# rslmtoasa/rslmtoasa

Hardware: AMD Instinct MI355X
Metric: block-recursion throughput (H|psi> + A_n + B_n recursion levels, recursion.f90 recur_b) (higher is better)
Workload: dtype f64

## Files before the change

include/rsrec.h:

```cpp
#ifndef RSREC_H
#define RSREC_H

#include <stddef.h>
#include <stdint.h>

#ifdef __cplusplus
extern "C" {
#endif

typedef struct rsrec_handle rsrec_t;

#define RSREC_OK 0
#define RSREC_ERR_ARG 1
#define RSREC_ERR_DEVICE 2
#define RSREC_ERR_DIVERGED 3
#define RSREC_ERR_EIG 4

int rsrec_version(void);

int rsrec_device_count(void);

int rsrec_create(rsrec_t **out, int device);
int rsrec_destroy(rsrec_t *h);

// ... 61 lines not shown

#define RSREC_LATTICE_NGROUP_MAX 16
int rsrec_chebyshev_lattice(rsrec_t *h, int nchains, int nseed, const int32_t *seed_atoms, const double *seed_coef, int lld, double a, double b,
                            int ngroup, const int32_t *group, double *m_g);

int rsrec_kubo_moments(rsrec_t *h, int nvec, int nseed, const int32_t *seed_atoms, const double *seed_coef, int cond_ll, double a, double b,
                       const double *v_a, const double *vo_a, const double *v_b, const double *vo_b, double *mu_nm);

int rsrec_kubo_moments_diag(rsrec_t *h, int nvec, int nseed, const int32_t *seed_atoms, const double *seed_coef, int cond_ll, double a, double b,
                            const double *v_a, const double *vo_a, const double *v_b, const double *vo_b, double *mu_diag);

#define RSREC_KUBO_NOUT_MAX 8
int rsrec_kubo_moments_diag_multi(rsrec_t *h, int nout, int nvec, int nseed, const int32_t *seed_atoms, const double *seed_coef,
                                  int cond_ll, double a, double b, const double *v_out, const double *vo_out, const double *v_b,
                                  const double *vo_b, double *mu_diag);

#define RSREC_KUBO_NIN_MAX 4
#define RSREC_KUBO_NSET_MAX 16
int rsrec_kubo_moments_diag_tensor(rsrec_t *h, int nin, int nout, int nvec, int nseed, const int32_t *seed_atoms, const double *seed_coef,
                                   int cond_ll, double a, double b, const double *v_out, const double *vo_out, const double *v_in,
                                   const double *vo_in, double *mu_diag);

#define RSREC_COND_LL_MAX 4096
int rsrec_kubo_integrand(rsrec_t *h, int nvec, int cond_ll, const double *mu_nm, int nen, const double *ene, double energy_min,
                         double energy_max, double *integrand);
int rsrec_kubo_integrand_diag(rsrec_t *h, int nvec, int cond_ll, const double *mu_diag, int nen, const double *ene, double energy_min,
                              double energy_max, double *integrand);

int rsrec_kubo_conductivity(rsrec_t *h, int nvec, int per_vector, int nen, int nv1, const double *ene, double energy_min, double energy_max,
                            double temperature, const double *integrand, double *sigma, double *series);

#define RSREC_OPT_NFERMI_MAX 16
int rsrec_kubo_optical(rsrec_t *h, int nset, int cond_ll, const double *mu_diag, int nen, const double *ene, double energy_min, double energy_max,
                       int nw, int nfermi, const double *fermi, double temperature, double *opt);

int rsrec_exchange(rsrec_t *h, int kind, int npairs, const int32_t *same, int lld, int nen, const double *ene, int nv1, double fermi,
                   int sym_term, double energy_min, double energy_max, const double *a_inf, const double *b_inf, const double *coef_a,
                   const double *coef_b, const double *dpar, int pair_offset, int npairs_total, double *xc, double *so, double *fo,
                   double *parts, double *jcum, double *integrand);

int rsrec_damping(rsrec_t *h, int kind, int npairs, const int32_t *same, int lld, int nen, const double *ene, int ief, int sym_term,
                  double energy_min, double energy_max, const double *a_inf, const double *b_inf, const double *coef_a, const double *coef_b,
                  const double *tmat, int pair_offset, int npairs_total, double *at_ef, double *total, double *rows);

int rsrec_exchange_aux(rsrec_t *h, int kind, int npairs, const int32_t *same, int lld, int nen, const double *ene, int nv1, double fermi,
                       int sym_term, double energy_min, double energy_max, const double *a_inf, const double *b_inf, const double *coef_a,
                       const double *coef_b, const double *apar, int pair_offset, int npairs_total, double *jaux, double *rows);

int rsrec_spin_lattice(rsrec_t *h, int kind, int npairs, const int32_t *same, int lld, int nen, const double *ene, int nv1, double fermi,
                       int sym_term, double energy_min, double energy_max, const double *a_inf, const double *b_inf, const double *coef_a,
                       const double *coef_b, const double *apar, const double *dmat, int trio_offset, int ntrios_total, double *jijk,
                       double *rows);

int rsrec_exchange_contour(rsrec_t *h, int kind, int npairs, const int32_t *same, int lld, int npts, const double *x, const double *w, double e0,
                           int sym_term, double energy_min, double energy_max, const double *a_inf, const double *b_inf, const double *coef_a,
                           const double *coef_b, const double *dmat, int pair_offset, int npairs_total, double *xc, double *rows);

int rsrec_contour_occupation(rsrec_t *h, int kind, int nsites, int lld, int npts, const double *x, const double *w, double e0, int sym_term,
                             double energy_min, double energy_max, const double *a_inf, const double *b_inf, const double *coef_a,
                             const double *coef_b, int site_offset, int nsites_total, double *occ, double *gdiag);

int rsrec_apply_operator(rsrec_t *h, int vel, const double *v_op, const double *vo_op, const double *psi_in, double *psi_out, double a, double b);

int rsrec_scalar_lanczos(rsrec_t *h, int nsites, const int32_t *seed_atoms, int lld, int llmax, double *a, double *b2);

void rsrec_site_partition(int rank, int nprocs, int nsites, int *start_atom, int *end_atom);

int rsrec_last_error(rsrec_t *h, char *buf, size_t n);

int rsrec_orbital_moments(rsrec_t *h, int nseeds, const int32_t *seed_atoms, int lld, double a, double b, const double *cr, double alat,
                          double *mu_orb, double *mu_seed);

int rsrec_pack_moments(rsrec_t *h, int site_offset, int nsites_total, double *mu_img);

#define RSREC_COMM_ID_BYTES 128
int rsrec_comm_unique_id(char *id);
int rsrec_comm_init(rsrec_t *h, int rank, int nranks, const char *id);
int rsrec_comm_init_file(rsrec_t *h, int rank, int nranks, const char *path, double timeout_s);
int rsrec_allreduce_sum(rsrec_t *h, double *buf, size_t n);
int rsrec_comm_size(rsrec_t *h, int *rank, int *nranks);
int rsrec_comm_destroy(rsrec_t *h);

int rsrec_set_option(rsrec_t *h, const char *key, long value);
int rsrec_get_timing(rsrec_t *h, double *out, int n);

#ifdef __cplusplus
}
#endif
#endif
```

rslmtoasa_amd/_lib.py:

```python
import ctypes as C
import os

_HERE = os.path.dirname(os.path.abspath(__file__))
LIB_PATH = os.environ.get("RSREC_LIB") or os.path.join(_HERE, "librsrec.so")

ERR_ARG, ERR_DEVICE, ERR_DIVERGED, ERR_EIG = 1, 2, 3, 4

_lib = None

_SIGNATURES = {
    "rsrec_version": (C.c_int, []),
    "rsrec_device_count": (C.c_int, []),
    "rsrec_create": (C.c_int, [C.POINTER(C.c_void_p), C.c_int]),
    "rsrec_destroy": (C.c_int, [C.c_void_p]),
    "rsrec_set_lattice": (C.c_int, [C.c_void_p, C.c_int, C.c_int, C.c_void_p, C.c_void_p, C.c_int, C.c_int]),
    "rsrec_set_positions": (C.c_int, [C.c_void_p, C.c_void_p]),
    "rsrec_set_hamiltonian": (C.c_int, [C.c_void_p, C.c_int, C.c_int, C.c_int] + [C.c_void_p] * 6),
    "rsrec_assemble_blocks": (C.c_int, [C.c_void_p, C.c_int, C.c_int, C.c_int, C.c_int, C.c_void_p, C.c_void_p, C.c_void_p, C.c_int, C.c_void_p, C.c_void_p]),
    "rsrec_block_lanczos": (C.c_int, [C.c_void_p, C.c_int, C.c_void_p, C.c_int, C.c_void_p, C.c_void_p]),
    "rsrec_block_lanczos_seeded": (C.c_int, [C.c_void_p, C.c_int, C.c_int, C.c_void_p, C.c_void_p, C.c_int, C.c_void_p, C.c_void_p]),
    "rsrec_block_lanczos_local_axis": (C.c_int, [C.c_void_p, C.c_int, C.c_void_p, C.c_void_p, C.c_int, C.c_void_p, C.c_void_p]),
    "rsrec_pack_diag": (C.c_int, [C.c_void_p, C.c_int, C.c_int, C.c_void_p, C.c_void_p]),
    "rsrec_orbital_moments": (C.c_int, [C.c_void_p, C.c_int, C.c_void_p, C.c_int, C.c_double, C.c_double, C.c_void_p, C.c_double, C.c_void_p, C.c_void_p]),
    "rsrec_pack_moments": (C.c_int, [C.c_void_p, C.c_int, C.c_int, C.c_void_p]),
    "rsrec_comm_unique_id": (C.c_int, [C.c_char_p]),
    "rsrec_comm_init": (C.c_int, [C.c_void_p, C.c_int, C.c_int, C.c_char_p]),
    "rsrec_comm_init_file": (C.c_int, [C.c_void_p, C.c_int, C.c_int, C.c_char_p, C.c_double]),
    "rsrec_allreduce_sum": (C.c_int, [C.c_void_p, C.c_void_p, C.c_size_t]),
    "rsrec_comm_size": (C.c_int, [C.c_void_p, C.POINTER(C.c_int), C.POINTER(C.c_int)]),
    "rsrec_comm_destroy": (C.c_int, [C.c_void_p]),
    "rsrec_terminator": (C.c_int, [C.c_void_p, C.c_int, C.c_int] + [C.c_void_p] * 6),
    "rsrec_scalar_density": (C.c_int, [C.c_void_p] + [C.c_int] * 4 + [C.c_void_p] * 2 + [C.c_int] + [C.c_void_p] * 4),
    "rsrec_block_ldos": (C.c_int, [C.c_void_p, C.c_int, C.c_void_p, C.c_double, C.c_double, C.c_int, C.c_int, C.c_int] + [C.c_void_p] * 5),
    "rsrec_kubo_moments": (C.c_int, [C.c_void_p, C.c_int, C.c_int, C.c_void_p, C.c_void_p, C.c_int, C.c_double, C.c_double] + [C.c_void_p] * 5),
    "rsrec_kubo_moments_diag": (C.c_int, [C.c_void_p, C.c_int, C.c_int, C.c_void_p, C.c_void_p, C.c_int, C.c_double, C.c_double] + [C.c_void_p] * 5),
    "rsrec_kubo_moments_diag_multi": (C.c_int, [C.c_void_p, C.c_int, C.c_int, C.c_int, C.c_void_p, C.c_void_p, C.c_int, C.c_double, C.c_double] + [C.c_void_p] * 5),
    "rsrec_kubo_moments_diag_tensor": (C.c_int, [C.c_void_p, C.c_int, C.c_int, C.c_int, C.c_int, C.c_void_p, C.c_void_p, C.c_int, C.c_double, C.c_double] + [C.c_void_p] * 5),
    "rsrec_exchange": (C.c_int, [C.c_void_p, C.c_int, C.c_int, C.c_void_p, C.c_int, C.c_int, C.c_void_p, C.c_int, C.c_double, C.c_int, C.c_double, C.c_double]
                       + [C.c_void_p] * 5 + [C.c_int, C.c_int] + [C.c_void_p] * 6),
    "rsrec_damping": (C.c_int, [C.c_void_p, C.c_int, C.c_int, C.c_void_p, C.c_int, C.c_int, C.c_void_p, C.c_int, C.c_int, C.c_double, C.c_double]
                      + [C.c_void_p] * 5 + [C.c_int, C.c_int] + [C.c_void_p] * 3),
    "rsrec_exchange_aux": (C.c_int, [C.c_void_p, C.c_int, C.c_int, C.c_void_p, C.c_int, C.c_int, C.c_void_p, C.c_int, C.c_double, C.c_int, C.c_double, C.c_double]
                           + [C.c_void_p] * 5 + [C.c_int, C.c_int] + [C.c_void_p] * 2),
    "rsrec_spin_lattice": (C.c_int, [C.c_void_p, C.c_int, C.c_int, C.c_void_p, C.c_int, C.c_int, C.c_void_p, C.c_int, C.c_double, C.c_int, C.c_double, C.c_double]
                           + [C.c_void_p] * 6 + [C.c_int, C.c_int] + [C.c_void_p] * 2),
    "rsrec_exchange_contour": (C.c_int, [C.c_void_p, C.c_int, C.c_int, C.c_void_p, C.c_int, C.c_int, C.c_void_p, C.c_void_p, C.c_double, C.c_int, C.c_double,
                                         C.c_double] + [C.c_void_p] * 5 + [C.c_int, C.c_int] + [C.c_void_p] * 2),
    "rsrec_contour_occupation": (C.c_int, [C.c_void_p, C.c_int, C.c_int, C.c_int, C.c_int, C.c_void_p, C.c_void_p, C.c_double, C.c_int, C.c_double,
                                           C.c_double] + [C.c_void_p] * 4 + [C.c_int, C.c_int] + [C.c_void_p] * 2),
    "rsrec_kubo_integrand": (C.c_int, [C.c_void_p, C.c_int, C.c_int, C.c_void_p, C.c_int, C.c_void_p, C.c_double, C.c_double, C.c_void_p]),
    "rsrec_kubo_integrand_diag": (C.c_int, [C.c_void_p, C.c_int, C.c_int, C.c_void_p, C.c_int, C.c_void_p, C.c_double, C.c_double, C.c_void_p]),
    "rsrec_kubo_conductivity": (C.c_int, [C.c_void_p, C.c_int, C.c_int, C.c_int, C.c_int, C.c_void_p, C.c_double, C.c_double, C.c_double] + [C.c_void_p] * 3),
    "rsrec_kubo_optical": (C.c_int, [C.c_void_p, C.c_int, C.c_int, C.c_void_p, C.c_int, C.c_void_p, C.c_double, C.c_double, C.c_int, C.c_int, C.c_void_p,
                                     C.c_double, C.c_void_p]),
    "rsrec_apply_operator": (C.c_int, [C.c_void_p, C.c_int, C.c_void_p, C.c_void_p, C.c_void_p, C.c_void_p, C.c_double, C.c_double]),
    "rsrec_zsqr": (C.c_int, [C.c_void_p, C.c_int, C.c_void_p]),
    "rsrec_chebyshev_green": (C.c_int, [C.c_void_p, C.c_int, C.c_int, C.c_int, C.c_void_p, C.c_double, C.c_double, C.c_void_p, C.c_void_p]),
    "rsrec_chebyshev_ldos": (C.c_int, [C.c_void_p, C.c_int, C.c_void_p, C.c_double, C.c_double, C.c_int, C.c_int] + [C.c_void_p] * 3),
    "rsrec_block_spectra": (C.c_int, [C.c_void_p, C.c_int, C.c_void_p, C.c_int, C.c_void_p, C.c_double, C.c_double, C.c_int, C.c_int, C.c_int, C.c_void_p]),
    "rsrec_chebyshev_spectra": (C.c_int, [C.c_void_p, C.c_int, C.c_void_p, C.c_int, C.c_void_p, C.c_double, C.c_double, C.c_int, C.c_int, C.c_void_p]),
    "rsrec_spectra_integrals": (C.c_int, [C.c_void_p, C.c_int, C.c_void_p, C.c_int, C.c_void_p, C.c_int, C.c_void_p, C.c_int, C.c_int, C.c_double, C.c_double,
                                          C.c_double, C.c_int, C.c_int, C.c_int, C.c_void_p, C.c_void_p]),
    "rsrec_block_green": (C.c_int, [C.c_void_p, C.c_int, C.c_int, C.c_int, C.c_void_p, C.c_double, C.c_double, C.c_int] + [C.c_void_p] * 5),
    "rsrec_chebyshev": (C.c_int, [C.c_void_p, C.c_int, C.c_void_p, C.c_int, C.c_double, C.c_double, C.c_void_p]),
    "rsrec_chebyshev_seeded": (C.c_int, [C.c_void_p, C.c_int, C.c_int, C.c_void_p, C.c_void_p, C.c_int, C.c_double, C.c_double, C.c_void_p]),
    "rsrec_chebyshev_pairs_direct": (C.c_int, [C.c_void_p, C.c_int, C.c_void_p, C.c_int, C.c_double, C.c_double, C.c_int, C.c_void_p, C.c_void_p]),
    "rsrec_chebyshev_bloch": (C.c_int, [C.c_void_p, C.c_int, C.c_void_p, C.c_int, C.c_double, C.c_double, C.c_void_p, C.c_void_p, C.c_int, C.c_void_p, C.c_int, C.c_void_p, C.c_void_p]),
    "rsrec_chebyshev_lattice": (C.c_int, [C.c_void_p, C.c_int, C.c_int, C.c_void_p, C.c_void_p, C.c_int, C.c_double, C.c_double, C.c_int, C.c_void_p, C.c_void_p]),
    "rsrec_scalar_lanczos":(C.c_int, [C.c_void_p, C.c_int, C.c_void_p, C.c_int, C.c_int, C.c_void_p, C.c_void_p]),
    "rsrec_site_partition": (None, [C.c_int, C.c_int, C.c_int, C.POINTER(C.c_int), C.POINTER(C.c_int)]),
    "rsrec_last_error": (C.c_int, [C.c_void_p, C.c_char_p, C.c_size_t]),
    "rsrec_set_option": (C.c_int, [C.c_void_p, C.c_char_p, C.c_long]),
    "rsrec_get_timing": (C.c_int, [C.c_void_p, C.POINTER(C.c_double), C.c_int]),
}


def exported_symbols():
    return sorted(_SIGNATURES)


def lib():
    global _lib
    if _lib is None:
        if not os.path.exists(LIB_PATH):
            raise RuntimeError("librsrec.so not built: run `make -C rslmtoasa_amd/csrc` (or __graft_entry__.build()); "
                               "there is no CPU fallback for the recursion engine")
        L = C.CDLL(LIB_PATH)
        for name, (res, args) in _SIGNATURES.items():
            fn = getattr(L, name)
            fn.restype = res
            fn.argtypes = args
        _lib = L
    return _lib


class RsrecError(RuntimeError):
    def __init__(self, code, msg):
        super().__init__("rsrec error %d: %s" % (code, msg))
        self.code = code
```

rslmtoasa_amd/csrc/kernels_uscheme.hpp:

```cpp
#pragma once
#include "kernels_mfma.hpp"
#include "kernels_spmm5.hpp"

namespace rsrec {

__host__ __device__ constexpr int pk_col(int q, int l4) { return q < 8 ? 8 * (q >> 1) + 2 * l4 + (q & 1) : 32 + l4; }

__device__ __forceinline__ void emit_rhs_frags_pk(const double2* M, double sign, double* out, int ci_layout) {
    for (int e = threadIdx.x; e < 27 * 64; e += blockDim.x) {
        const int l = e & 63, qf = e >> 6, q = qf / 3, f = qf % 3;
        const int ki = pk_col(q, l >> 4);
        const int ko = (f < 2) ? 16 * f + (l & 15) : 32 + (l & 3);
        const int pi = ci_layout ? (ki & 1) : ki / 18, ci = ci_layout ? (ki >> 1) : ki % 18;
        const int po = ci_layout ? (ko & 1) : ko / 18, co = ci_layout ? (ko >> 1) : ko % 18;
        const double2 g = M[ci + 18 * co];
        const double v = (pi == po) ? g.x : (pi == 0 ? g.y : -g.y);
        out[e] = sign * v;
    }
}

__device__ __forceinline__ void matmul18(const double2* A, const double2* B, double2* C) {
    for (int e = threadIdx.x; e < BLK; e += blockDim.x) {
        const int i = e % NB, j = e / NB;
        double2 acc = make_double2(0.0, 0.0);
        for (int k = 0; k < NB; ++k) {
            const double2 a = A[i + NB * k], b = B[k + NB * j];
            acc.x += a.x * b.x - a.y * b.y;
            acc.y += a.x * b.y + a.y * b.x;
        }
        C[e] = acc;
    }
}

struct U3Operands { double2 x[4]; double2 y; };

__device__ __forceinline__ void u3_load(U3Operands& o, const double* __restrict__ base, unsigned off, int l4) {
    const double2* p = reinterpret_cast<const double2*>(base + off + 2 * l4);
#pragma unroll
    for (int qq = 0; qq < 4; ++qq) o.x[qq] = ld_stream(p + 4 * qq);
    o.y = ld_stream(reinterpret_cast<const double2*>(base + off + 32 + 2 * (l4 >> 1)));
}

template <int Q>
__device__ __forceinline__ double u3_k(const U3Operands& o, bool odd) { return Q < 8 ? ((Q & 1) ? o.x[Q >> 1].y : o.x[Q >> 1].x) : (odd ? o.y.y : o.y.x); }

__device__ __forceinline__ void u3_mac(double4_t& ca, double4_t& cb, double& cr, const U3Operands& o, const double (&T)[27], bool odd) {
#define U3_STEP(Q)                                                                              \
    {                                                                                           \
        const double a = u3_k<Q>(o, odd);                                                          \
        ca = __builtin_amdgcn_mfma_f64_16x16x4f64(a, T[3 * (Q) + 0], ca, 0, 0, 0);              \
        cb = __builtin_amdgcn_mfma_f64_16x16x4f64(a, T[3 * (Q) + 1], cb, 0, 0, 0);              \
        cr = __builtin_amdgcn_mfma_f64_4x4x4f64(a, T[3 * (Q) + 2], cr, 0, 0, 0);                \
    }
    U3_STEP(0) U3_STEP(1) U3_STEP(2) U3_STEP(3) U3_STEP(4) U3_STEP(5) U3_STEP(6) U3_STEP(7) U3_STEP(8)
#undef U3_STEP
}

__global__ __launch_bounds__(MF_WAVES * 64, 1) void k_mfma_orth3(ChainView CV, int level, int zero_block, const double* __restrict__ tvec,
                                                                const double* __restrict__ ucur, double* uprev,
                                                                const double* __restrict__ tabs, double* partial ,
                                                                double* unext = nullptr ) {
    __shared__ double lds[MF_WAVES * 1296];
    const int chain = blockIdx.y;
    const int lane = threadIdx.x & 63;
    const int wave = __builtin_amdgcn_readfirstlane(threadIdx.x >> 6);
    const int ngroups = CV.count_of(chain, level) / GROUP;
    const int* order = CV.order_of(chain, level);
    const size_t vo = (size_t)chain * CV.vstride;
    const double* tv = tvec + vo;
    const double* uc = ucur + vo;
    double* up = uprev + vo;
    double* uo = (unext ? unext : uprev) + vo;
    const int l15 = lane & 15, l4 = lane >> 4, l3 = lane & 3, lg = (lane >> 2) & 3;
    double T1[27], T2[27], T3[27];
    {
        const double* f = tabs + (size_t)chain * 3 * 27 * 64 + lane;
#pragma unroll
        for (int e = 0; e < 27; ++e) { T1[e] = f[e * 64]; T2[e] = f[(27 + e) * 64]; T3[e] = f[(54 + e) * 64]; }
    }
    GramAcc Gm;
    Gm.zero();
    const int nbx = active_workgroups(ngroups);
    GroupWalk w((int)blockIdx.x < nbx ? ngroups : 0, wave, nbx);
    const int ntile = (w.g < w.end) ? ((w.end - w.g + w.step - 1) / w.step) * 9 : 0;
    struct TileAtoms { int s0, a_lo, a_hi; };
    auto tile_atoms = [&](int it) {
        it = min(it, ntile - 1);
        const int* __restrict__ grp = order + (size_t)(w.g + (it / 9) * w.step) * GROUP;
        TileAtoms t;
        t.s0 = (16 * (it % 9)) / 18;
        t.a_lo = grp[t.s0];
        t.a_hi = grp[min(t.s0 + 1, GROUP - 1)];
        return t;
    };
    auto tile_row = [&](const TileAtoms& t, int rho) {
        const bool hi = rho >= 18 * (t.s0 + 1);
        const int a = hi ? t.a_hi : t.a_lo;
        RowRef R;
        R.valid = a >= 0;
        R.off = (unsigned)BLD * (unsigned)(R.valid ? a : zero_block) + 36u * (unsigned)(rho - 18 * (t.s0 + (hi ? 1 : 0)));
        return R;
    };
    auto load_tile = [&](int it, U3Operands& a, U3Operands& c, U3Operands& p) {
        const TileAtoms t = tile_atoms(it);
        const RowRef ra = tile_row(t, 16 * (min(it, ntile - 1) % 9) + l15);
        u3_load(a, tv, ra.off, l4);
        u3_load(c, uc, ra.off, l4);
        u3_load(p, up, ra.off, l4);
    };
    struct Pending { double4_t ca, cb; double cr; TileAtoms ta; int mt; };
    Pending P;
    bool pending = false;
    auto retire = [&](const double (&fr)[4]) {
#pragma unroll
        for (int j = 0; j < 4; ++j) {
            const RowRef rs = tile_row(P.ta, 16 * P.mt + l4 + 4 * j);
            if (rs.valid) { st_stream(uo + rs.off + l15, (double)P.ca[j]); st_stream(uo + rs.off + 16 + l15, (double)P.cb[j]); }
        }
        const RowRef rr = tile_row(P.ta, 16 * P.mt + 4 * lg + l4);
        if (rr.valid) st_stream(uo + rr.off + 32 + l3, P.cr);
#pragma unroll
        for (int j = 0; j < 4; ++j) {
            const double f0 = P.ca[j], f1 = P.cb[j];
            Gm.t00 = __builtin_amdgcn_mfma_f64_16x16x4f64(f0, f0, Gm.t00, 0, 0, 0);
            Gm.t01 = __builtin_amdgcn_mfma_f64_16x16x4f64(f0, f1, Gm.t01, 0, 0, 0);
            Gm.t11 = __builtin_amdgcn_mfma_f64_16x16x4f64(f1, f1, Gm.t11, 0, 0, 0);
            Gm.tr0 = __builtin_amdgcn_mfma_f64_4x4x4f64(fr[j], f0, Gm.tr0, 0, 0, 0);
            Gm.tr1 = __builtin_amdgcn_mfma_f64_4x4x4f64(fr[j], f1, Gm.tr1, 0, 0, 0);
            Gm.trr = __builtin_amdgcn_mfma_f64_4x4x4f64(fr[j], fr[j], Gm.trr, 0, 0, 0);
        }
    };
    auto compute_tile = [&](int it, const U3Operands& ot, const U3Operands& oc, const U3Operands& op) {
        double fr[4] = {0.0, 0.0, 0.0, 0.0};
        if (pending) {
#pragma unroll
            for (int j = 0; j < 4; ++j) fr[j] = __shfl(P.cr, l3 + 4 * j + 16 * l4, 64);
        }
        Pending N;
        N.ta = tile_atoms(it);
        N.mt = it % 9;
        N.ca = (double4_t){0, 0, 0, 0}; N.cb = (double4_t){0, 0, 0, 0}; N.cr = 0.0;
        u3_mac(N.ca, N.cb, N.cr, ot, T1, l4 & 1);
        if (pending) retire(fr);
        u3_mac(N.ca, N.cb, N.cr, op, T2, l4 & 1);
        u3_mac(N.ca, N.cb, N.cr, oc, T3, l4 & 1);
        P = N;
        pending = true;
    };
    U3Operands at, ac, ap, bt, bc, bp, ct, cc, cp;
    if (ntile > 0) { load_tile(0, at, ac, ap); load_tile(1, bt, bc, bp); }
#pragma unroll 1
    for (int it = 0; it < ntile; it += 3) {
        load_tile(it + 2, ct, cc, cp);
        __builtin_amdgcn_sched_barrier(0);
        compute_tile(it, at, ac, ap);
        __builtin_amdgcn_sched_barrier(0);
        if (it + 1 < ntile) {
            load_tile(it + 3, at, ac, ap);
            __builtin_amdgcn_sched_barrier(0);
            compute_tile(it + 1, bt, bc, bp);
            __builtin_amdgcn_sched_barrier(0);
        }
        if (it + 2 < ntile) {
            load_tile(it + 4, bt, bc, bp);
            __builtin_amdgcn_sched_barrier(0);
            compute_tile(it + 2, ct, cc, cp);
            __builtin_amdgcn_sched_barrier(0);
        }
    }
    if (pending) {
        double fr[4];
#pragma unroll
        for (int j = 0; j < 4; ++j) fr[j] = __shfl(P.cr, l3 + 4 * j + 16 * l4, 64);
        retire(fr);
    }
    gram_block_out(Gm, lds, partial + ((size_t)chain * gridDim.x + blockIdx.x) * 1296, true);
}

template <int F>
__device__ __forceinline__ void u3_mac_lds(double4_t& ca, double4_t& cb, double& cr, const U3Operands& o, const double* __restrict__ T , bool odd) {
#define U3L_STEP(Q)                                                                             \
    {                                                                                           \
        const double a = u3_k<Q>(o, odd);                                                          \
        ca = __builtin_amdgcn_mfma_f64_16x16x4f64(a, T[(3 * (Q) + 0) * 64], ca, 0, 0, 0);       \
        cb = __builtin_amdgcn_mfma_f64_16x16x4f64(a, T[(3 * (Q) + 1) * 64], cb, 0, 0, 0);       \
        cr = __builtin_amdgcn_mfma_f64_4x4x4f64(a, T[(3 * (Q) + 2) * 64], cr, 0, 0, 0);         \
    }
    U3L_STEP(0) U3L_STEP(1) U3L_STEP(2) U3L_STEP(3) U3L_STEP(4) U3L_STEP(5) U3L_STEP(6) U3L_STEP(7) U3L_STEP(8)
#undef U3L_STEP
}

__global__ __launch_bounds__(MF_WAVES * 64, 2) void k_mfma_orth3w(ChainView CV, int level, int zero_block, const double* __restrict__ tvec,
                                                                 const double* __restrict__ ucur, double* uprev,
                                                                 const double* __restrict__ tabs, double* partial ) {
    __shared__ double lds[MF_WAVES * 1296];
    const int chain = blockIdx.y;
    const int lane = threadIdx.x & 63;
    const int wave = __builtin_amdgcn_readfirstlane(threadIdx.x >> 6);
    const int ngroups = CV.count_of(chain, level) / GROUP;
    const int* order = CV.order_of(chain, level);
    const size_t vo = (size_t)chain * CV.vstride;
    const double* tv = tvec + vo;
    const double* uc = ucur + vo;
// ... 271 lines not shown
```

rslmtoasa_amd/csrc/rsrec.hip:

```cpp
#include <hip/hip_runtime.h>
#include <hsa/hsa.h>
#include <hsa/hsa_ext_amd.h>
#include <dlfcn.h>
#include <algorithm>
#include <array>
#include <atomic>
#include <chrono>
#include <cmath>
#include <cstdarg>
#include <cstdio>
#include <cstdlib>
#include <cstring>
#include <memory>
#include <string>
#include <thread>
#include <tuple>
#include <vector>

#include "../../include/rsrec.h"
#include "kernels_valu.hpp"
#include "kernels_mfma.hpp"
#include "kernels_spmm4.hpp"
#include "kernels_spmm5.hpp"
#include "kernels_uscheme.hpp"
#include "kernels_green.hpp"
#include "kernels_ldos.hpp"
#include "kernels_spectra.hpp"
#include "kernels_moments.hpp"
#include "kernels_kubo.hpp"
#include "kernels_cond.hpp"
#include "kernels_optical.hpp"
#include "kernels_exchange.hpp"
#include "kernels_auxgreen.hpp"
#include "kernels_contour.hpp"
#include "kernels_assemble.hpp"
#include "kernels_fan.hpp"
#include "kernels_bloch.hpp"
#include "kernels_lattice.hpp"

using namespace rsrec;

namespace {

struct DevBuf {
    void* p = nullptr;
    size_t bytes = 0;
    DevBuf() = default;
    DevBuf(DevBuf&& o) noexcept : p(o.p), bytes(o.bytes) { o.p = nullptr; o.bytes = 0; }
    DevBuf& operator=(DevBuf&& o) noexcept { std::swap(p, o.p); std::swap(bytes, o.bytes); return *this; }
    ~DevBuf() { release(); }
    hipError_t reserve(size_t n) {
        if (n <= bytes) return hipSuccess;
        release();
        hipError_t e = hipMalloc(&p, n);
        if (e == hipSuccess) bytes = n;
        return e;
    }
    void release() { if (p) (void)hipFree(p); p = nullptr; bytes = 0; }
    template <class T> T* as() const { return reinterpret_cast<T*>(p); }
};

}

struct rsrec_handle {
    int device = 0;
    hipStream_t stream = nullptr;
    hipStream_t copy_stream = nullptr;
    hipEvent_t ev_green[2] = {nullptr, nullptr};
    hipStream_t side_stream = nullptr;
    hipEvent_t ev_orth = nullptr, ev_bred = nullptr;
    hipStream_t oct_stream = nullptr;
    hipEvent_t ev_oct_in = nullptr, ev_oct_out = nullptr;
    size_t p2_slot = 0;
    std::string err;
    bool have_lattice = false, have_ham = false;
    std::vector<int32_t> lat_nn, lat_iz;
    int lat_nncols = 0;
    std::vector<double> lat_cr;
    int kk = 0, nslots = 0, nmax = 0, ntype = 0;
    std::vector<int> nbr;
    std::vector<int> iz0;
    std::vector<int> radj_ptr, radj;
    DevBuf d_nbr, d_iz, d_nbr5;
    int hslots = 0, hoh = 0, nsp = 2;
    DevBuf d_hst, d_hloc, d_host, d_holoc, d_enim, d_lsham;
    Spmm4Operator s4_op;
    int s4_built_split = 0;
    Spmm5Operator s5_op;
    DevBuf d_s5queue;
    int s5_built = 0;
    size_t s5_lds_limit = (size_t)-1;
    int n_cu = 0;
    bool s4_attr = false;
    size_t term_lds = 0, cheb_ldos_lds = (size_t)64 * 1024, cheb_spec_lds = (size_t)64 * 1024;
    std::vector<double> host_ee, host_lsham, host_eeo, host_enim, host_hall, host_hallo;
    std::vector<double> host_st, host_loc;
    DevBuf d_asm[2][2], d_asm_in;
    std::vector<double> asm_host[2][2];
    int asm_nslots[2] = {0, 0}, asm_ncls[2] = {0, 0}, asm_hoh[2] = {0, 0};
    int n_octet_launch = 0;
    int n_asm_reused = 0;
    long n_asm_calls = 0, n_ldos_calls = 0, n_recursion_calls = 0;
    Spmm5Operator s5_la; int s5_la_ok = 0;
    DevBuf d_la_extra, d_rot;
    Spmm5Operator kubo_op[RSREC_KUBO_NOUT_MAX], kubo_op_b[RSREC_KUBO_NIN_MAX], kubo_hbulk;
    Spmm5Operator orb_plain;
    DevBuf d_green_in, d_green_out;
    DevBuf d_kubo[5];
    DevBuf d_cond[4];
    DevBuf d_ctens[2];
    DevBuf d_opt[5];
    DevBuf d_bsqrt, d_term, d_gim, d_ldos;
    DevBuf d_ops, d_spec;
    struct SpecImage { int nop = 0, nen = 0, n = 0, site_offset = 0, nsites_total = 0; } spec_res;
    DevBuf d_mint;
    void* pin = nullptr;
    size_t pin_bytes = 0;
    DevBuf d_frags, d_vec[6], d_partial, d_partial2, d_coefA, d_coefB, d_bmats, d_status, d_seed, d_seedcoef, d_mu, d_scal, d_zsqr;
    DevBuf d_fan, d_fan_tab, d_mpair;
    DevBuf d_bloch_geo, d_bloch_tab;
    DevBuf d_lat_tab, d_lat_w, d_lat_part;
    long opt_batch = 0, opt_kernels = 0, opt_nblk = 0, opt_spmm5 = 2, opt_chain_fold = 1, opt_s5_cap = 0, opt_side = 1, opt_s5_lds = 1, opt_s5_queue = 1, opt_cheb_fused = 1;
    long opt_s5_waves = 8;
    long opt_sat_pct = 100;
    long opt_orth_oop = 1;
    long opt_s5_split = 0;
    long opt_s5_run_min = 0;
    long opt_s5_spin_xcd = 0;
    long opt_s5_octet = 8;
    long opt_s5_host_emit = 0;
    long opt_kubo_lchunk = 0;
    long opt_kubo_vbatch = 0;
    long opt_lattice_vbatch = 0;
    long opt_kubo_setgroup = 0;
    int n_kubo_left_chunks = 0;
    int kubo_diag_nvec = 0, kubo_diag_ll = 0;
    long opt_orth3 = 1;
    long opt_graph = 1;
    long opt_s5_gram_min = 256;
    int ham_hermitian = 0;
    std::vector<int> opp_slot;
    int opp_epoch = -1;
    DevBuf d_gram;
    double n_gram_folded = 0, n_gram_all = 0, n_gram_levels = 0;
    hipGraphExec_t graph_exec = nullptr;
    std::vector<uintptr_t> graph_key;
    bool capturing = false;
    double t_total_ms = 0, t_hop_ms = 0, t_rest_ms = 0, t_host_ms = 0;
    double t_rot_ms = 0;
    double n_hop_launch = 0, n_atom_steps = 0, n_block_mult = 0, n_hop_mfma_flop = 0;
    double n_req_flop = 0;
    int hop_fuses_a = 1;
    std::vector<hipEvent_t> ev_pool;
    size_t ev_used = 0;
    struct RegionEntry {
        std::vector<int> seeds;
        int nlev, napply, flags, epoch, ostride;
        double atom_steps, block_mults;
        DevBuf order, cum;
        std::vector<int> level_max;
        std::vector<int> hop_min, hop_max;
        std::vector<double> level_groups;
        std::vector<double> mult_hist;
        struct ClassRun { int tau, lo, hi; };
        std::vector<ClassRun> sat_runs;
        std::vector<int> level_sat;
        int sat_base = 0;
    };
    std::vector<std::unique_ptr<RegionEntry>> region_cache;
    int lattice_epoch = 0;
    const int* cur_order = nullptr;
    const int* cur_cum = nullptr;
    const std::vector<int>* cur_level_max = nullptr;
    const std::vector<double>* cur_level_groups = nullptr;
    const std::vector<double>* cur_mult_hist = nullptr;
    const RegionEntry* cur_entry = nullptr;
    int cur_nrows = 0;
    std::vector<unsigned> spatial_key;
    int res_kind = 0, res_n = 0, res_lld = 0;
    bool res_seeded = false;
    void* comm = nullptr;
    int comm_rank = 0, comm_nranks = 1;
    DevBuf d_comm;
    ~rsrec_handle();
};

namespace {

struct OptionEntry { const char* name; long rsrec_handle::*member; };
const OptionEntry OPTIONS[] = {
    {"batch", &rsrec_handle::opt_batch},
    {"kernels", &rsrec_handle::opt_kernels},
    {"nblk", &rsrec_handle::opt_nblk},
    {"spmm5", &rsrec_handle::opt_spmm5},
    {"chain_fold", &rsrec_handle::opt_chain_fold},
    {"s5_cap", &rsrec_handle::opt_s5_cap},
    {"s5_lds", &rsrec_handle::opt_s5_lds},
    {"s5_queue", &rsrec_handle::opt_s5_queue},
    {"cheb_fused", &rsrec_handle::opt_cheb_fused},
    {"side_stream", &rsrec_handle::opt_side},
    {"graph", &rsrec_handle::opt_graph},
    {"orth3", &rsrec_handle::opt_orth3},
    {"s5_waves", &rsrec_handle::opt_s5_waves},
    {"s5_split", &rsrec_handle::opt_s5_split},
    {"orth_oop", &rsrec_handle::opt_orth_oop},
    {"sat_pct", &rsrec_handle::opt_sat_pct},
    {"kubo_lchunk", &rsrec_handle::opt_kubo_lchunk},
    {"kubo_vbatch", &rsrec_handle::opt_kubo_vbatch},
    {"kubo_setgroup", &rsrec_handle::opt_kubo_setgroup},
    {"lattice_vbatch", &rsrec_handle::opt_lattice_vbatch},
    {"s5_host_emit", &rsrec_handle::opt_s5_host_emit},
    {"s5_octet", &rsrec_handle::opt_s5_octet},
    {"s5_spin_xcd", &rsrec_handle::opt_s5_spin_xcd},
    {"s5_run_min", &rsrec_handle::opt_s5_run_min},
    {"s5_gram_min", &rsrec_handle::opt_s5_gram_min},
};

int fail(rsrec_t* h, int code, const char* fmt, ...) {
    char buf[512];
    va_list ap;
    va_start(ap, fmt);
    vsnprintf(buf, sizeof buf, fmt, ap);
    va_end(ap);
    if (h) h->err = buf;
    return code;
}

#define HIPCK(h, call)                                                                                         \
    do {                                                                                                       \
        hipError_t e_ = (call);                                                                                \
        if (e_ != hipSuccess) return fail(h, RSREC_ERR_DEVICE, "%s failed: %s (%s:%d)", #call, hipGetErrorString(e_), __FILE__, __LINE__); \
    } while (0)

hipEvent_t next_event(rsrec_t* h) {
    static const bool off = getenv("RSREC_NO_EVENTS") != nullptr;
    if (off || h->capturing) return nullptr;
    if (h->ev_used == h->ev_pool.size()) {
        hipEvent_t e;
        if (hipEventCreate(&e) != hipSuccess) return nullptr;
        h->ev_pool.push_back(e);
    }
    hipEvent_t e = h->ev_pool[h->ev_used++];
    (void)hipEventRecord(e, h->stream);
    return e;
}

constexpr size_t PIN_BYTES = (size_t)8 << 20;
int pin_ready(rsrec_t* h) {
    if (h->pin) return RSREC_OK;
    if (hipHostMalloc(&h->pin, PIN_BYTES, hipHostMallocDefault) != hipSuccess) { h->pin = nullptr; return fail(h, RSREC_ERR_DEVICE, "hipHostMalloc of the staging buffer failed"); }
    h->pin_bytes = PIN_BYTES;
    return RSREC_OK;
}
constexpr size_t PIN_MAX_XFER = (size_t)8 << 20;
int xfer_d2h(rsrec_t* h, void* dst, const void* src_dev, size_t bytes) {
    if (bytes > PIN_MAX_XFER) {
        HIPCK(h, hipMemcpyAsync(dst, src_dev, bytes, hipMemcpyDeviceToHost, h->stream));
        HIPCK(h, hipStreamSynchronize(h->stream));
        return RSREC_OK;
    }
    int rc = pin_ready(h);
    if (rc) return rc;
    for (size_t off = 0; off < bytes; off += h->pin_bytes) {
        const size_t n = std::min(h->pin_bytes, bytes - off);
        HIPCK(h, hipMemcpyAsync(h->pin, static_cast<const char*>(src_dev) + off, n, hipMemcpyDeviceToHost, h->stream));
        HIPCK(h, hipStreamSynchronize(h->stream));
        memcpy(static_cast<char*>(dst) + off, h->pin, n);
    }
    return RSREC_OK;
}
int xfer_h2d(rsrec_t* h, void* dst_dev, const void* src, size_t bytes) {
    if (bytes > PIN_MAX_XFER) {
        HIPCK(h, hipMemcpyAsync(dst_dev, src, bytes, hipMemcpyHostToDevice, h->stream));
        HIPCK(h, hipStreamSynchronize(h->stream));
        return RSREC_OK;
    }
    int rc = pin_ready(h);
    if (rc) return rc;
    for (size_t off = 0; off < bytes; off += h->pin_bytes) {
        const size_t n = std::min(h->pin_bytes, bytes - off);
        memcpy(h->pin, static_cast<const char*>(src) + off, n);
        HIPCK(h, hipMemcpyAsync(static_cast<char*>(dst_dev) + off, h->pin, n, hipMemcpyHostToDevice, h->stream));
        HIPCK(h, hipStreamSynchronize(h->stream));
    }
    return RSREC_OK;
}
#define XFER(call) do { int rc__ = (call); if (rc__) return rc__; } while (0)

// ... 60 lines not shown
void spatial_key_from_graph(rsrec_t* h) {
    const int kk = h->kk;
    std::vector<int> d0, d1, d2;
    bfs_dist(h, 0, d0);
    int l1 = 0;
    for (int i = 0; i < kk; ++i) if (d0[i] >= d0[l1]) l1 = i;
    bfs_dist(h, l1, d1);
    int l2 = 0, best = -1;
    for (int i = 0; i < kk; ++i) { const int m = std::min(d0[i], d1[i]); if (m >= best) { best = m; l2 = i; } }
    bfs_dist(h, l2, d2);
    h->spatial_key.resize(kk);
    for (int i = 0; i < kk; ++i) h->spatial_key[i] = morton3((unsigned)std::max(d0[i], 0), (unsigned)std::max(d1[i], 0), (unsigned)std::max(d2[i], 0));
}

}

extern "C" int rsrec_version(void) { return 101; }

extern "C" int rsrec_device_count(void) {
    int n = 0;
    if (hipGetDeviceCount(&n) != hipSuccess) return 0;
    return n;
}

static rsrec_handle* g_report_handle = nullptr;
static void report_at_exit() {
    const rsrec_handle* h = g_report_handle;
    if (!h) return;
    std::printf("rsrec report: library_calls=%ld device_assemblies=%ld operator_arrays_from_device=%d device_ldos_calls=%ld\n", h->n_recursion_calls, h->n_asm_calls,
                h->n_asm_reused, h->n_ldos_calls);
    std::fflush(stdout);
}

extern "C" int rsrec_create(rsrec_t** out, int device) {
    if (!out) return RSREC_ERR_ARG;
    *out = nullptr;
    int ndev = 0;
    if (hipGetDeviceCount(&ndev) != hipSuccess || ndev <= 0) return RSREC_ERR_DEVICE;
    if (device < 0 || device >= ndev) return RSREC_ERR_ARG;
    if (hipSetDevice(device) != hipSuccess) return RSREC_ERR_DEVICE;
    rsrec_t* h = new rsrec_handle();
    h->device = device;
    if (hipStreamCreateWithFlags(&h->stream, hipStreamNonBlocking) != hipSuccess) { delete h; return RSREC_ERR_DEVICE; }
    if (hipDeviceGetAttribute(&h->n_cu, hipDeviceAttributeMultiprocessorCount, device) != hipSuccess || h->n_cu <= 0) h->n_cu = 256;
    *out = h;
    if (getenv("RSREC_REPORT") && !g_report_handle) {
        static bool registered = false;
        if (!registered) { registered = std::atexit(report_at_exit) == 0; }
        g_report_handle = h;
    }
    return RSREC_OK;
}

rsrec_handle::~rsrec_handle() {
    (void)hipSetDevice(device);
    if (stream) (void)hipStreamSynchronize(stream);
    if (graph_exec) (void)hipGraphExecDestroy(graph_exec);
    (void)rsrec_comm_destroy(this);
    for (hipEvent_t e : ev_pool) (void)hipEventDestroy(e);
    for (hipStream_t s : {stream, copy_stream, side_stream, oct_stream}) if (s) (void)hipStreamDestroy(s);
    for (hipEvent_t e : {ev_green[0], ev_green[1], ev_orth, ev_bred, ev_oct_in, ev_oct_out}) if (e) (void)hipEventDestroy(e);
    if (pin) (void)hipHostFree(pin);
}

extern "C" int rsrec_destroy(rsrec_t* h) {
    if (!h) return RSREC_ERR_ARG;
    if (g_report_handle == h) { report_at_exit(); g_report_handle = nullptr; }
    delete h;
    return RSREC_OK;
}

extern "C" int rsrec_last_error(rsrec_t* h, char* buf, size_t n) {
    if (!h || !buf || n == 0) return RSREC_ERR_ARG;
    snprintf(buf, n, "%s", h->err.c_str());
    return RSREC_OK;
}

extern "C" int rsrec_set_option(rsrec_t* h, const char* key, long value) {
    if (!h || !key) return RSREC_ERR_ARG;
    for (const OptionEntry& o : OPTIONS)
        if (!strcmp(key, o.name)) { h->*o.member = value; return RSREC_OK; }
    return fail(h, RSREC_ERR_ARG, "unknown option '%s'", key);
}

extern "C" int rsrec_get_timing(rsrec_t* h, double* out, int n) {
    if (!h || !out) return RSREC_ERR_ARG;
    const double v[14] = {h->t_total_ms, h->t_hop_ms, h->n_hop_launch, h->n_atom_steps, h->n_block_mult, h->t_rest_ms, h->t_host_ms, (double)h->hop_fuses_a, h->n_hop_mfma_flop,
                          h->n_req_flop, (double)h->n_asm_reused, (double)h->n_octet_launch, h->t_rot_ms, h->n_gram_folded};
    for (int i = 0; i < n && i < 14; ++i) out[i] = v[i];
    return RSREC_OK;
}

extern "C" void rsrec_site_partition(int rank, int nprocs, int nsites, int* start_atom, int* end_atom) {
    int per = nsites / nprocs;
    const int rem = nsites % nprocs;
    int start;
    if (rank < rem) { per += 1; start = rank * per + 1; }
    else start = rank * per + rem + 1;
    *start_atom = start;
    *end_atom = start + per - 1;
}

static void release_graph(rsrec_t* h) {
    if (h->graph_exec) { (void)hipDeviceSynchronize(); (void)hipGraphExecDestroy(h->graph_exec); h->graph_exec = nullptr; }
    h->graph_key.clear();
}

static void release_regions(rsrec_t* h) {
    release_graph(h);
    if (!h->region_cache.empty()) (void)hipDeviceSynchronize();
    h->region_cache.clear();
    h->cur_order = nullptr; h->cur_cum = nullptr; h->cur_entry = nullptr; h->cur_level_max = nullptr; h->cur_level_groups = nullptr; h->cur_mult_hist = nullptr;
}

extern "C" int rsrec_set_lattice(rsrec_t* h, int kk, int nncols, const int32_t* nn, const int32_t* iz, int nmax, int ntype) {
    if (!h || !nn || !iz || kk <= 0 || nncols < 1 || nmax < 0 || nmax > kk || ntype < 1) return fail(h, RSREC_ERR_ARG, "rsrec_set_lattice: bad argument");
    HIPCK(h, hipSetDevice(h->device));
    if (h->have_lattice && kk == h->kk && nncols == h->lat_nncols && nmax == h->nmax && ntype == h->ntype &&
        h->lat_nn.size() == (size_t)kk * nncols && std::memcmp(h->lat_nn.data(), nn, h->lat_nn.size() * sizeof(int32_t)) == 0 &&
        std::memcmp(h->lat_iz.data(), iz, (size_t)kk * sizeof(int32_t)) == 0)
        return RSREC_OK;
    int nslots = 1;
    for (int i = 0; i < kk; ++i) {
        const int nr = nn[i];
        if (nr < 0 || nr > nncols) return fail(h, RSREC_ERR_ARG, "rsrec_set_lattice: nn(%d,1)=%d outside 0..%d", i + 1, nr, nncols);
        nslots = std::max(nslots, nr);
        if (iz[i] < 1 || iz[i] > ntype) return fail(h, RSREC_ERR_ARG, "rsrec_set_lattice: iz(%d)=%d outside 1..%d", i + 1, iz[i], ntype);
    }
    std::vector<int> nbr_new((size_t)kk * nslots, -1), iz_new(kk), deg(kk + 1, 0);
    for (int i = 0; i < kk; ++i) {
        iz_new[i] = iz[i] - 1;
        nbr_new[(size_t)i * nslots] = i;
        const int nr = nn[i];
        for (int j = 1; j < nr; ++j) {
            const int n = nn[(size_t)i + (size_t)kk * j];
            if (n == 0) continue;
            if (n < 0 || n > kk) return fail(h, RSREC_ERR_ARG, "rsrec_set_lattice: nn(%d,%d)=%d outside 0..%d", i + 1, j + 1, n, kk);
            nbr_new[(size_t)i * nslots + j] = n - 1;
            deg[n - 1]++;
        }
    }
    h->have_lattice = false;
    h->have_ham = false;
    h->kubo_diag_nvec = h->kubo_diag_ll = 0;
    h->lat_nn.clear(); h->lat_iz.clear();
    release_regions(h);
    h->kk = kk; h->nslots = nslots; h->nmax = nmax; h->ntype = ntype;
    h->nbr.swap(nbr_new);
    h->iz0.swap(iz_new);
    h->radj_ptr.assign(kk + 1, 0);
    for (int n = 0; n < kk; ++n) h->radj_ptr[n + 1] = h->radj_ptr[n] + deg[n];
    h->radj.resize(h->radj_ptr[kk]);
    std::vector<int> fill(h->radj_ptr.begin(), h->radj_ptr.end() - 1);
    for (int i = 0; i < kk; ++i)
        for (int j = 1; j < nslots; ++j) {
            const int n = h->nbr[(size_t)i * nslots + j];
            if (n >= 0) h->radj[fill[n]++] = i;
        }
    HIPCK(h, h->d_nbr.reserve(h->nbr.size() * sizeof(int)));
    HIPCK(h, h->d_iz.reserve((size_t)kk * sizeof(int)));
    HIPCK(h, hipMemcpy(h->d_nbr.p, h->nbr.data(), h->nbr.size() * sizeof(int), hipMemcpyHostToDevice));
    HIPCK(h, hipMemcpy(h->d_iz.p, h->iz0.data(), (size_t)kk * sizeof(int), hipMemcpyHostToDevice));
    {
        std::vector<int> n5((size_t)(kk + 1) * (nslots + 2), kk);
        for (int i = 0; i < kk; ++i) {
            for (int j = 0; j < nslots; ++j) { const int n = h->nbr[(size_t)i * nslots + j]; if (n >= 0) n5[(size_t)i * (nslots + 2) + j] = n; }
// ... 121 lines not shown
        if (dev && !hoh) k_fold_onsite<<<ntype, 324, 0, h->stream>>>(h->d_hst.as<double2>(), nslots, h->d_lsham.as<double2>(), nullptr);
    }
    std::vector<double> loc;
    if (nmax > 0) {
        loc.assign(hall, hall + B * nslots * nmax);
        if (!hoh)
            for (int i = 0; i < nmax; ++i)
                for (size_t e = 0; e < B; ++e) loc[B * nslots * i + e] += lsham[B * h->iz0[i] + e];
        const double* dev = resident(1, 0, hall, nmax);
        HIPCK(h, place(h->d_hloc, dev, loc.data(), loc.size()));
        if (dev && !hoh) k_fold_onsite<<<nmax, 324, 0, h->stream>>>(h->d_hloc.as<double2>(), nslots, h->d_lsham.as<double2>(), h->d_iz.as<int>());
    }
    if (hoh) {
        HIPCK(h, place(h->d_host, resident(0, 1, eeo, ntype), eeo, B * nslots * ntype));
        HIPCK(h, h->d_enim.reserve(B * ntype * 8));
        HIPCK(h, hipMemcpy(h->d_enim.p, enim, B * ntype * 8, hipMemcpyHostToDevice));
        if (nmax > 0) HIPCK(h, place(h->d_holoc, resident(1, 1, hallo, nmax), hallo, B * nslots * nmax));
    }
    HIPCK(h, hipGetLastError());
    {
        h->s4_built_split = 0; h->s5_built = 0;
        if (h->nslots + 1 <= S4_MAXSLOTS) {
            h->host_st.swap(st);
            h->host_loc.swap(loc);
            const double* dev[6] = {h->d_hst.as<double>(), h->d_hloc.as<double>(), h->d_host.as<double>(), h->d_holoc.as<double>(), h->d_enim.as<double>(), h->d_lsham.as<double>()};
            const char* msg = h->s5_op.build(h->nslots, nslots, ntype, nmax, h->hoh, h->host_st.data(), nmax > 0 ? h->host_loc.data() : nullptr, hoh ? eeo : nullptr,
                                             (hoh && nmax > 0) ? hallo : nullptr, hoh ? enim : nullptr, lsham, h->iz0.data(), h->opt_s5_host_emit ? nullptr : dev, h->stream);
            if (msg) return fail(h, RSREC_ERR_DEVICE, "rsrec_set_hamiltonian: %s", msg);
            h->s5_built = 1;
        }
    }
    h->have_ham = true;
    return RSREC_OK;
}

extern "C" int rsrec_assemble_blocks(rsrec_t* h, int part, int ncls, int nslots, int hoh, const double* hmag, const int32_t* nbr_type, const double* obarm, int ntype,
                                     double* blocks, double* blocks_o) {
    if (!h) return RSREC_ERR_ARG;
    if (part < 0 || part > 1 || ncls < 1 || nslots < 1 || !hmag || !blocks) return fail(h, RSREC_ERR_ARG, "rsrec_assemble_blocks: part=%d ncls=%d nslots=%d or a missing array", part, ncls, nslots);
    if (hoh && (!nbr_type || !obarm || !blocks_o || ntype < 1)) return fail(h, RSREC_ERR_ARG, "rsrec_assemble_blocks: hoh needs nbr_type, obarm (ntype=%d) and blocks_o", ntype);
    if (hoh)
        for (size_t q = 0; q < (size_t)ncls * nslots; ++q)
            if (nbr_type[q] < 0 || nbr_type[q] > ntype) return fail(h, RSREC_ERR_ARG, "rsrec_assemble_blocks: nbr_type[%zu]=%d outside 0..%d", q, nbr_type[q], ntype);
    HIPCK(h, hipSetDevice(h->device));
    h->n_asm_calls++;
    h->asm_nslots[part] = h->asm_ncls[part] = 0;
    const size_t nblk = (size_t)ncls * nslots, hm_bytes = nblk * 4 * 81 * 16, ty_bytes = nblk * 4, ob_bytes = hoh ? (size_t)ntype * 324 * 16 : 0;
    const size_t ty_off = (hm_bytes + 255) / 256 * 256, ob_off = ty_off + (ty_bytes + 255) / 256 * 256;
    HIPCK(h, h->d_asm_in.reserve(ob_off + ob_bytes + 256));
    char* in = h->d_asm_in.as<char>();
    XFER(xfer_h2d(h, in, hmag, hm_bytes));
    if (hoh) { XFER(xfer_h2d(h, in + ty_off, nbr_type, ty_bytes)); XFER(xfer_h2d(h, in + ob_off, obarm, ob_bytes)); }
    HIPCK(h, h->d_asm[part][0].reserve(nblk * 324 * 16));
    if (hoh) HIPCK(h, h->d_asm[part][1].reserve(nblk * 324 * 16));
    k_assemble_blocks<<<dim3(nslots, ncls), 384, 0, h->stream>>>(reinterpret_cast<const double2*>(in), reinterpret_cast<const int*>(in + ty_off),
                                                                 reinterpret_cast<const double2*>(in + ob_off), nslots, hoh ? 1 : 0, h->d_asm[part][0].as<double2>(),
                                                                 hoh ? h->d_asm[part][1].as<double2>() : nullptr);
    HIPCK(h, hipGetLastError());
    XFER(xfer_d2h(h, blocks, h->d_asm[part][0].p, nblk * 324 * 16));
    if (hoh) XFER(xfer_d2h(h, blocks_o, h->d_asm[part][1].p, nblk * 324 * 16));
    h->asm_host[part][0].assign(blocks, blocks + nblk * 648);
    if (hoh) h->asm_host[part][1].assign(blocks_o, blocks_o + nblk * 648); else h->asm_host[part][1].clear();
    h->asm_nslots[part] = nslots; h->asm_ncls[part] = ncls; h->asm_hoh[part] = hoh ? 1 : 0;
    return RSREC_OK;
}

namespace {

DevProblem make_problem(const rsrec_t* h) {
    DevProblem P;
    P.kk = h->kk; P.nslots = h->nslots; P.hstride = h->hslots; P.nmax = h->nmax; P.hoh = h->hoh;
    P.nbr = h->d_nbr.as<int>(); P.iz = h->d_iz.as<int>();
    P.h_st = h->d_hst.as<double2>(); P.h_loc = h->d_hloc.as<double2>();
    P.ho_st = h->d_host.as<double2>(); P.ho_loc = h->d_holoc.as<double2>();
    P.enim = h->d_enim.as<double2>(); P.lsham = h->d_lsham.as<double2>();
    return P;
}

void release_kubo_buffers(rsrec_t* h, bool moments, bool integrand) {
    if (moments) { for (auto& kb : h->d_kubo) kb.release(); h->kubo_diag_nvec = h->kubo_diag_ll = 0; }
    if (integrand) { for (auto& cb : h->d_cond) cb.release(); for (auto& cb : h->d_ctens) cb.release(); for (auto& cb : h->d_opt) cb.release(); }
}

struct BatchPlan {
    int batch = 1, nblk = 1;
};

int plan_batch(rsrec_t* h, int nchains, int nvec, size_t vec_elems_per_chain, BatchPlan& bp, size_t extra_bytes_per_chain = 0) {
    release_kubo_buffers(h, true, true);
    size_t free_b = 0, total_b = 0;
    HIPCK(h, hipMemGetInfo(&free_b, &total_b));
    size_t reusable = 0;
    for (int v = 0; v < 5; ++v) reusable += h->d_vec[v].bytes;
    if (extra_bytes_per_chain) reusable += h->d_gram.bytes;
    const double per_chain = (double)nvec * vec_elems_per_chain * sizeof(double2) + (double)h->kk * 4 + 4096 + (double)extra_bytes_per_chain;
    long cap = (long)((0.85 * (double)(free_b + reusable)) / per_chain);
    if (cap < 1) return fail(h, RSREC_ERR_DEVICE, "not enough device memory for one chain (%.1f MB needed, %.1f MB free)", per_chain / 1e6, free_b / 1e6);
    long b = h->opt_batch > 0 ? h->opt_batch : 64;
    b = std::min<long>(b, cap);
    b = std::min<long>(b, nchains);
    bp.batch = (int)std::max<long>(b, 1);
    long nblk = h->opt_nblk > 0 ? h->opt_nblk : std::max<long>(2048 / bp.batch, 16);
    nblk = std::min<long>(nblk, 256);
    nblk = std::min<long>(nblk, (h->kk + TILE_ATOMS - 1) / TILE_ATOMS);
    bp.nblk = (int)std::max<long>(nblk, 1);
    return RSREC_OK;
}

int upload_regions(rsrec_t* h, const int* seeds0, int nb, int nseed, int nlev, int napply, bool two_pass, bool grouped, int& ostride,
                   double& atom_steps, double& block_mults) {
    const int kk = h->kk;
    const int cap = grouped ? kk + 7 * h->nmax + 7 * h->ntype + 8 : kk;
    const int cap_pre = ((grouped ? kk + 7 * h->nmax + 7 * h->ntype * nlev + 8 : kk) + GROUP - 1) / GROUP * GROUP;
    const int flags = (two_pass ? 1 : 0) | (grouped ? 2 : 0) | ((int)std::min<long>(100, std::max<long>(1, h->opt_sat_pct)) << 2) | (nseed << 9);
    for (const auto& e : h->region_cache)
        if (e->epoch == h->lattice_epoch && e->nlev == nlev && e->napply == napply && e->flags == flags && (int)e->seeds.size() == nb * nseed &&
            std::equal(e->seeds.begin(), e->seeds.end(), seeds0)) {
            h->cur_order = e->order.as<int>(); h->cur_cum = e->cum.as<int>(); h->cur_nrows = nb; h->cur_level_max = &e->level_max; h->cur_level_groups = &e->level_groups;
            h->cur_mult_hist = &e->mult_hist;
            h->cur_entry = e.get();
            ostride = e->ostride;
            atom_steps += e->atom_steps; block_mults += e->block_mults;
            return RSREC_OK;
        }
    const int ntau_h = h->nmax + h->ntype, nfs_h = h->nslots + 1;
    const int sat_pct = (int)std::min<long>(100, std::max<long>(1, h->opt_sat_pct));
    const int sat_from = (int)(((long)sat_pct * kk + 99) / 100);
    std::vector<Region> regs(nb);
    auto run_threads = [&](auto&& fn) {
        const int nthr = std::max(1, std::min({nb, 8, (int)std::thread::hardware_concurrency()}));
        if (nthr == 1) { for (int c = 0; c < nb; ++c) fn(c); return; }
        std::atomic<int> next_chain{0};
        std::vector<std::thread> pool;
        for (int t = 0; t < nthr; ++t)
            pool.emplace_back([&]() { for (int c = next_chain++; c < nb; c = next_chain++) fn(c); });
        for (auto& th : pool) th.join();
    };
    run_threads([&](int c) { grow_region(h, seeds0 + (size_t)c * nseed, nseed, nlev, regs[c]); });
    size_t lvneed = 8;
    for (int c = 0; c < nb; ++c) {
        size_t need = 0;
        for (int L = 0; L < nlev; ++L) {
            const int n = regs[c].cum[L];
            if (n >= sat_from || (L > 0 && n == regs[c].cum[L - 1])) continue;
            need += (size_t)n + (grouped ? (size_t)7 * std::min(ntau_h, n) + 8 : 0);
        }
        lvneed = std::max(lvneed, need);
    }
    lvneed = (lvneed + 7) / 8 * 8;
    if (lvneed + (size_t)cap > (size_t)INT32_MAX) return fail(h, RSREC_ERR_ARG, "region lists of %zu entries per chain exceed the index range", lvneed + (size_t)cap);
    if ((size_t)cap_pre + lvneed + (size_t)cap > (size_t)INT32_MAX) return fail(h, RSREC_ERR_ARG, "region lists of %zu entries per chain exceed the index range", (size_t)cap_pre + lvneed + (size_t)cap);
    const int sat_off = cap_pre + (int)lvneed;
    ostride = sat_off + cap;
    std::vector<int> order((size_t)nb * ostride, -1), cum((size_t)4 * nb * nlev, 0);
    std::vector<double> as(nb, 0.0), bm(nb, 0.0);
    const size_t hist_n = (size_t)2 * ntau_h * nfs_h;
    std::vector<double> hist((size_t)nb * hist_n, 0.0);
    auto tau = [&](int i) { return i < h->nmax ? i : h->nmax + h->iz0[i]; };
    const std::vector<unsigned>& key = h->spatial_key;
    auto before = [&](int x, int y) {
        const int tx = grouped ? tau(x) : 0, ty = grouped ? tau(y) : 0;
        if (tx != ty) return tx < ty;
        if (key[x] != key[y]) return key[x] < key[y];
        return x < y;
    };
    std::vector<int> all(kk), sat_list;
    for (int i = 0; i < kk; ++i) all[i] = i;
    std::sort(all.begin(), all.end(), before);
    sat_list.reserve(cap);
    for (int q = 0; q < kk; ++q) {
        if (grouped && q > 0 && tau(all[q]) != tau(all[q - 1])) while (sat_list.size() % GROUP) sat_list.push_back(-1);
        sat_list.push_back(all[q]);
    }
    if (grouped) while (sat_list.size() % GROUP) sat_list.push_back(-1);
    const int sat_count = (int)sat_list.size();
    std::vector<double> lgroups((size_t)nb * nlev * ntau_h, 0.0);
    auto build_chain = [&](int c) {
        const Region& R = regs[c];
        int* orow = order.data() + (size_t)c * ostride;
        int* crow = cum.data() + (size_t)c * nlev;
        int* brow = cum.data() + (size_t)(nb + c) * nlev;
        int* crow2 = cum.data() + (size_t)(2 * nb + c) * nlev;
        int* brow2 = cum.data() + (size_t)(3 * nb + c) * nlev;
        std::copy(sat_list.begin(), sat_list.end(), orow + sat_off);
        int w = cap_pre, wp = 0;
        std::vector<int> lev, region, merged;
        for (int L = 0; L < nlev; ++L) {
            const int lo = L ? R.cum[L - 1] : 0, hi = R.cum[L];
            if (hi >= sat_from) { crow[L] = crow2[L] = sat_count; brow[L] = brow2[L] = sat_off; continue; }
            lev.assign(R.order.begin() + lo, R.order.begin() + hi);
            std::sort(lev.begin(), lev.end(), before);
            for (size_t q = 0; q < lev.size(); ++q) {
                if (grouped && q > 0 && tau(lev[q]) != tau(lev[q - 1])) while (wp % GROUP) orow[wp++] = -1;
                orow[wp++] = lev[q];
            }
            if (grouped) while (wp % GROUP) orow[wp++] = -1;
            crow2[L] = wp; brow2[L] = 0;
            if (L > 0 && hi == lo) { crow[L] = crow[L - 1]; brow[L] = brow[L - 1]; continue; }
            merged.resize(region.size() + lev.size());
            std::merge(region.begin(), region.end(), lev.begin(), lev.end(), merged.begin(), before);
            region.swap(merged);
            brow[L] = w;
            double* G = lgroups.data() + ((size_t)c * nlev + L) * ntau_h;
            for (size_t q = 0; q < region.size(); ++q) {
                if (grouped && q > 0 && tau(region[q]) != tau(region[q - 1])) while (w % GROUP) orow[w++] = -1;
                if (w % GROUP == 0) G[grouped ? tau(region[q]) : 0] += 1.0;
                orow[w++] = region[q];
            }
            if (grouped) while (w % GROUP) orow[w++] = -1;
            crow[L] = w - brow[L];
        }
        double a_s = 0.0, b_m = 0.0;
        for (int t = 1; t <= napply; ++t) {
            const int lv_after = two_pass ? 2 * t : t;
            a_s += R.cum[std::min(lv_after, nlev - 1)];
        }
        std::vector<int> lev_of(kk, -1);
        {
            int lv = 0;
            for (int q = 0; q < R.cum[nlev - 1]; ++q) {
                while (q >= R.cum[lv]) ++lv;
                lev_of[R.order[q]] = lv;
            }
        }
        std::vector<double> uses1(nlev + 1, 0.0), uses2(nlev + 1, 0.0);
        for (int d = 0; d < nlev; ++d)
            for (int t = 1; t <= napply; ++t) {
                if (!two_pass) { if (d <= t - 1) uses1[d] += 1.0; }
                else { if (d <= 2 * (t - 1)) uses1[d] += 1.0; if (d <= 2 * t - 1) uses2[d] += 1.0; }
            }
        double* H = hist.data() + (size_t)c * hist_n;
        const int ns = h->nslots;
        for (int i = 0; i < kk; ++i) {
            const int ti = tau(i);
            for (int s = 0; s < ns; ++s) {
                const int n = h->nbr[(size_t)i * ns + s];
                if (n < 0 || lev_of[n] < 0) continue;
                H[(size_t)ti * nfs_h + s] += uses1[lev_of[n]];
                if (two_pass) H[((size_t)ntau_h + ti) * nfs_h + s] += uses2[lev_of[n]];
            }
            if (two_pass && lev_of[i] >= 0) H[((size_t)ntau_h + ti) * nfs_h + ns] += uses1[lev_of[i]];
        }
        for (size_t q = 0; q < hist_n; ++q) b_m += H[q];
        if (two_pass) for (int t2 = 0; t2 < ntau_h; ++t2) b_m += H[((size_t)ntau_h + t2) * nfs_h + ns];
        as[c] = a_s; bm[c] = b_m;
    };
    run_threads(build_chain);
    double as_sum = 0.0, bm_sum = 0.0;
    for (int c = 0; c < nb; ++c) { as_sum += as[c]; bm_sum += bm[c]; }
    atom_steps += as_sum; block_mults += bm_sum;
    if (h->region_cache.size() >= 256) {
        HIPCK(h, hipStreamSynchronize(h->stream));
        h->region_cache.clear();
        h->cur_entry = nullptr;
    }
    h->region_cache.push_back(std::make_unique<rsrec_handle::RegionEntry>());
    rsrec_handle::RegionEntry* e = h->region_cache.back().get();
    e->seeds.assign(seeds0, seeds0 + (size_t)nb * nseed);
    e->nlev = nlev; e->napply = napply; e->flags = flags; e->epoch = h->lattice_epoch; e->ostride = ostride;
    e->atom_steps = as_sum; e->block_mults = bm_sum;
    e->mult_hist.assign(hist_n, 0.0);
    for (int c = 0; c < nb; ++c)
        for (size_t q = 0; q < hist_n; ++q) e->mult_hist[q] += hist[(size_t)c * hist_n + q];
    HIPCK(h, e->order.reserve(order.size() * 4));
    HIPCK(h, e->cum.reserve(cum.size() * 4));
    XFER(xfer_h2d(h, e->order.p, order.data(), order.size() * 4));
    XFER(xfer_h2d(h, e->cum.p, cum.data(), cum.size() * 4));
    HIPCK(h, hipStreamSynchronize(h->stream));
    e->level_max.assign(nlev, 0);
    e->hop_min.assign(nlev, INT32_MAX); e->hop_max.assign(nlev, 0);
    e->level_groups.assign((size_t)nlev * ntau_h, 0.0);
    {
        std::vector<double> sat_hist(ntau_h, 0.0);
        for (int g = 0; g < sat_count / GROUP; ++g) sat_hist[tau(sat_list[(size_t)g * GROUP])] += 1.0;
        e->sat_base = sat_off;
        e->level_sat.assign(nlev, 0);
        if (grouped)
            for (int g = 0; g < sat_count / GROUP; ++g) {
                const int t = tau(sat_list[(size_t)g * GROUP]);
                if (e->sat_runs.empty() || e->sat_runs.back().tau != t) e->sat_runs.push_back({t, g, g + 1});
                else e->sat_runs.back().hi = g + 1;
            }
        for (int c = 0; c < nb; ++c) {
            const double* prev = nullptr;
            for (int l = 0; l < nlev; ++l) {
                const int cnt = cum[(size_t)c * nlev + l];
                e->level_max[l] = std::max(e->level_max[l], cnt);
                e->hop_min[l] = std::min(e->hop_min[l], cnt); e->hop_max[l] = std::max(e->hop_max[l], cnt);
                const bool sat = cum[(size_t)(nb + c) * nlev + l] == sat_off;
                e->level_max[l] = std::max(e->level_max[l], cum[(size_t)(2 * nb + c) * nlev + l]);
                if (sat) e->level_sat[l] += 1;
                const double* G = lgroups.data() + ((size_t)c * nlev + l) * ntau_h;
                if (!sat && l > 0 && cum[(size_t)(nb + c) * nlev + l] == cum[(size_t)(nb + c) * nlev + l - 1] && prev) G = prev;
                for (int t2 = 0; t2 < ntau_h; ++t2) e->level_groups[(size_t)l * ntau_h + t2] += sat ? sat_hist[t2] : G[t2];
                prev = sat ? nullptr : G;
            }
        }
    }
    h->cur_order = e->order.as<int>(); h->cur_cum = e->cum.as<int>(); h->cur_nrows = nb; h->cur_level_max = &e->level_max; h->cur_level_groups = &e->level_groups;
    h->cur_mult_hist = &e->mult_hist;
    h->cur_entry = e;
    return RSREC_OK;
}

double required_hop_flops(const rsrec_t* h, const Spmm5Operator& op) {
    if (!h->cur_mult_hist) return 0.0;
    const int ntau = h->nmax + h->ntype, nfs = h->nslots + 1;
    const std::vector<double>& H = *h->cur_mult_hist;
    if (H.size() != (size_t)2 * ntau * nfs) return 0.0;
    double f = 0.0;
    for (int pass = 0; pass < 2; ++pass)
        for (int t = 0; t < ntau; ++t)
            for (int s = 0; s < nfs; ++s) {
                const double n = H[((size_t)pass * ntau + t) * nfs + s];
                if (n == 0.0) continue;
                const double w = (op.mixing.empty() || op.ntau != ntau || op.nslots != h->nslots) ? 46656.0 : op.required_flops(pass, t, s);
                f += n * (w > 0.0 ? w : 46656.0);
            }
    return f;
}

void reset_timing(rsrec_t* h) {
    h->t_total_ms = h->t_hop_ms = h->t_rest_ms = h->t_host_ms = h->t_rot_ms = 0;
    h->n_hop_launch = h->n_atom_steps = h->n_block_mult = h->n_hop_mfma_flop = h->n_req_flop = 0;
    h->n_octet_launch = 0;
    h->n_gram_folded = h->n_gram_all = h->n_gram_levels = 0;
    h->ev_used = 0;
    h->n_recursion_calls++;
}

// ... 239 lines not shown
int ensure_s4(rsrec_t* h) {
    if (h->s4_built_split) return RSREC_OK;
    const char* msg = h->s4_op.build(h->nslots, h->hslots, h->ntype, h->nmax, 0, h->host_st.data(), h->nmax > 0 ? h->host_loc.data() : nullptr, nullptr, nullptr, 1);
    if (msg) return fail(h, RSREC_ERR_DEVICE, "k_spmm4 operator tables: %s", msg);
    h->s4_built_split = 1;
    return RSREC_OK;
}

int s4_prepare(rsrec_t* h) {
    if (!h->s4_attr) {
        HIPCK(h, hipFuncSetAttribute(reinterpret_cast<const void*>(k_spmm4<4>), hipFuncAttributeMaxDynamicSharedMemorySize, (int)S4_LDS_BYTES));
        h->s4_attr = true;
    }
    return RSREC_OK;
}
int launch_spmm(rsrec_t* h, const SpmmDims& SD, const ChainView& CV, const DevProblem& P, int set, const double* in, double* out, dim3 grid_mf) {
    { const int rc = s4_prepare(h); if (rc) return rc; }
    dim3 g4(std::min<unsigned>(grid_mf.x * 4, 1024), grid_mf.y);
    k_spmm4<4><<<g4, MF_WAVES * 64, S4_LDS_BYTES, h->stream>>>(SD, CV.order, CV.cum, P.nbr, P.iz, h->s4_op.frag_set(set), h->s4_op.meta_set(set), in, out);
    return RSREC_OK;
}

__global__ __launch_bounds__(256) void k_rotate_coef(double2* __restrict__ A, double2* __restrict__ B, const double2* __restrict__ rot, int lld) {
#pragma clang fp contract(off)
    __shared__ double2 sM[BLK], sR[BLK], sT[BLK];
    const int chain = blockIdx.y, m = blockIdx.x;
    const bool is_a = m < lld - 1;
    double2* M = (is_a ? A : B) + ((size_t)chain * lld + (is_a ? m : m - (lld - 1) + 1)) * BLK;
    const double2* R = rot + (size_t)chain * BLK;
    for (int e = threadIdx.x; e < BLK; e += blockDim.x) { sM[e] = M[e]; sR[e] = R[e]; }
    __syncthreads();
    for (int e = threadIdx.x; e < BLK; e += blockDim.x) {
        const int i = e % NB, j = e / NB;
        double sr = 0.0, si = 0.0;
#pragma unroll
        for (int k = 0; k < NB; ++k) {
            const double ar = sM[i + NB * k].x, ai = sM[i + NB * k].y, br = sR[k + NB * j].x, bi = sR[k + NB * j].y;
            sr += ar * br - ai * bi; si += ar * bi + ai * br;
        }
        sT[e] = make_double2(sr, si);
    }
    __syncthreads();
    for (int e = threadIdx.x; e < BLK; e += blockDim.x) {
        const int i = e % NB, j = e / NB;
        double sr = 0.0, si = 0.0;
#pragma unroll
        for (int k = 0; k < NB; ++k) {
            const double ar = sR[k + NB * i].x, ai = -sR[k + NB * i].y, br = sT[k + NB * j].x, bi = sT[k + NB * j].y;
            sr += ar * br - ai * bi; si += ar * bi + ai * br;
        }
        M[e] = make_double2(sr, si);
    }
}

struct RecursionCall {
    bool mfma = false, side = false;
    int nchains = 0, nseed = 1, napply = 0, nlev = 0;
    const double* rot = nullptr;
    const Spmm5Operator* op = nullptr;
    int ci = 0;
    size_t velems = 0;
    int nvec = 0, skip_vec = -1, B = 1, nblk = 1;
    DevProblem P;
    hipEvent_t ev_begin = nullptr;
    std::vector<std::pair<hipEvent_t, hipEvent_t>> hop_ev, rot_ev;
};

RecursionCall recursion_call(const rsrec_t* h, bool mfma, int nchains, int nseed, int napply, const double* rot = nullptr) {
    RecursionCall RC;
    RC.mfma = mfma; RC.nchains = nchains; RC.nseed = nseed; RC.napply = napply; RC.rot = rot;
    RC.nlev = (h->hoh ? 2 * napply : napply) + 1; RC.op = rot ? &h->s5_la : &h->s5_op; RC.velems = (size_t)(h->kk + 1) * BLD;
    const bool large = (long)std::min(nchains, 64) * (h->kk / GROUP + 1) >= 4096;
    RC.ci = (mfma && (h->hoh || rot || h->opt_spmm5 == 2 || (h->opt_spmm5 == 1 && large) || !spmm4_usable(h))) ? 1 : 0;
    return RC;
}

bool matrix_core_set(const rsrec_t* h) { return h->opt_kernels != 1 && h->s5_built; }
void drop_resident(rsrec_t* h) { h->res_kind = 0; h->spec_res.nop = 0; }

int recursion_begin(rsrec_t* h, RecursionCall& RC, int nvec, int skip_vec, int coef_slots, size_t gram_doubles_per_chain = 0) {
    if (RC.mfma && !RC.ci) XFER(ensure_s4(h));
    RC.nvec = nvec; RC.skip_vec = skip_vec;
    BatchPlan bp;
    XFER(plan_batch(h, RC.nchains, nvec - (skip_vec >= 0 ? 1 : 0), RC.velems / 2, bp, gram_doubles_per_chain * sizeof(double)));
    const int B = RC.B = bp.batch; RC.nblk = bp.nblk;
    for (int v = 0; v < nvec; ++v) if (v != skip_vec) HIPCK(h, h->d_vec[v].reserve((size_t)B * RC.velems * sizeof(double)));
    if (gram_doubles_per_chain) HIPCK(h, h->d_gram.reserve((size_t)B * gram_doubles_per_chain * sizeof(double)));
    XFER(reserve_partials(h, B, (size_t)B * 256 * 2 * 1296 * sizeof(double)));
    XFER(ensure_side_stream(h));
    RC.side = h->opt_side && h->side_stream;
    if (RC.rot) HIPCK(h, h->d_la_extra.reserve((size_t)B * (h->nmax + h->ntype) * S5_HEAD_DOUBLES * sizeof(double)));
    HIPCK(h, h->d_status.reserve(64));
    HIPCK(h, h->d_seed.reserve((size_t)B * RC.nseed * 4));
    HIPCK(h, h->d_seedcoef.reserve((size_t)B * coef_slots * sizeof(double2)));
    HIPCK(h, hipMemsetAsync(h->d_status.p, 0, 64, h->stream));
    RC.P = make_problem(h); RC.ev_begin = next_event(h);
    return RSREC_OK;
}

void local_axis_fragments(const rsrec_t* h, const Spmm5Operator& OP, const double* rot, int c0, int nb, std::vector<double>& fr) {
    const bool hoh = h->hoh != 0;
    const int ntau = h->nmax + h->ntype, la_fps = S5_HEAD_DOUBLES;
    std::vector<double> E(2 * BLK), T(2 * BLK); fr.assign((size_t)nb * ntau * la_fps, 0.0);
    for (int c = 0; c < nb; ++c) {
        const double* R = rot + 2 * (size_t)BLK * (c0 + c);
        for (int tau = 0; tau < ntau; ++tau) {
            const int ty = tau < h->nmax ? h->iz0[tau] : tau - h->nmax;
            const double* ls = h->host_lsham.data() + 2 * (size_t)BLK * ty;
            for (int j = 0; j < NB; ++j)
                for (int i = 0; i < NB; ++i) {
                    double sr = 0.0, si = 0.0;
                    for (int k = 0; k < NB; ++k) {
                        const double ar = ls[2 * (i + NB * k)], ai = ls[2 * (i + NB * k) + 1], br = R[2 * (j + NB * k)], bi = -R[2 * (j + NB * k) + 1];
                        sr += ar * br - ai * bi; si += ar * bi + ai * br;
                    }
                    T[2 * (i + NB * j)] = sr; T[2 * (i + NB * j) + 1] = si;
                }
            for (int j = 0; j < NB; ++j)
                for (int i = 0; i < NB; ++i) {
                    double sr = 0.0, si = 0.0;
                    for (int k = 0; k < NB; ++k) {
                        const double ar = R[2 * (i + NB * k)], ai = R[2 * (i + NB * k) + 1], br = T[2 * (k + NB * j)], bi = T[2 * (k + NB * j) + 1];
                        sr += ar * br - ai * bi; si += ar * bi + ai * br;
                    }
                    E[2 * (i + NB * j)] = sr; E[2 * (i + NB * j) + 1] = si;
                }
            if (hoh) for (int e = 0; e < 2 * BLK; ++e) E[e] += h->host_enim[2 * (size_t)BLK * ty + e];
            OP.emit_head(hoh ? 1 : 0, tau, E.data(), fr.data() + ((size_t)c * ntau + tau) * la_fps);
        }
    }
}

struct RecursionBatch {
    int nb = 0, ostride = 0;
    ChainView CV, CVp;
    dim3 grid_mf;
    const double* la_extra = nullptr;
};
using SeedCoefHook = void (*)(int nb, int nseed, const std::vector<int>& seeds0, std::vector<double>& coef);
int recursion_batch(rsrec_t* h, const RecursionCall& RC, const int32_t* seed_atoms, const double* seed_coef, int c0, int nb, RecursionBatch& b,
                    SeedCoefHook extra_coef = nullptr) {
    const auto th0 = std::chrono::steady_clock::now();
    std::vector<int> seeds0;
    std::vector<double> coef, fr;
    stage_seeds(seed_atoms, seed_coef, c0, nb, RC.nseed, seeds0, coef);
    if (extra_coef) extra_coef(nb, RC.nseed, seeds0, coef);
    b.nb = nb; b.ostride = h->kk;
    XFER(upload_regions(h, seeds0.data(), nb, RC.nseed, RC.nlev, RC.napply, h->hoh != 0, RC.mfma, b.ostride, h->n_atom_steps, h->n_block_mult));
    h->n_req_flop += required_hop_flops(h, *RC.op);
    XFER(xfer_h2d(h, h->d_seed.p, seeds0.data(), seeds0.size() * 4));
    XFER(xfer_h2d(h, h->d_seedcoef.p, coef.data(), coef.size() * 8));
    if (RC.rot) {
        local_axis_fragments(h, *RC.op, RC.rot, c0, nb, fr);
        XFER(xfer_h2d(h, h->d_la_extra.p, fr.data(), fr.size() * sizeof(double)));
        b.la_extra = h->d_la_extra.as<double>();
    }
    HIPCK(h, hipStreamSynchronize(h->stream));
    h->t_host_ms += std::chrono::duration<double, std::milli>(std::chrono::steady_clock::now() - th0).count();
    chain_views(h, RC.nlev, RC.velems, 1, b.ostride, b.CV, &b.CVp);
    b.grid_mf = dim3(std::max(1, std::min(mfma_workgroups_per_chain(h, RC.B), (b.ostride / GROUP + MF_WAVES - 1) / MF_WAVES)), nb);
    return RSREC_OK;
}

int clear_vectors(rsrec_t* h, const RecursionCall& RC, int nb, int zero_block_only = -1) {
    for (int v = 0; v < RC.nvec; ++v) {
        if (v == RC.skip_vec) continue;
        if (v == zero_block_only)
            HIPCK(h, hipMemset2DAsync(static_cast<char*>(h->d_vec[v].p) + (size_t)h->kk * BLD * sizeof(double), RC.velems * sizeof(double), 0, BLD * sizeof(double), (size_t)nb, h->stream));
        else HIPCK(h, hipMemsetAsync(h->d_vec[v].p, 0, (size_t)nb * RC.velems * sizeof(double), h->stream));
// ... 92 lines not shown
    if (!h->graph_exec || key != h->graph_key) {
        if (h->graph_exec) { (void)hipGraphExecDestroy(h->graph_exec); h->graph_exec = nullptr; }
        h->graph_key.clear();
        s5_prepare(h);
        XFER(s4_prepare(h));
        HIPCK(h, hipStreamSynchronize(h->stream));
        HIPCK(h, hipStreamBeginCapture(h->stream, hipStreamCaptureModeRelaxed));
        h->capturing = true;
        const int rc = enqueue();
        h->capturing = false;
        hipGraph_t graph = nullptr;
        const hipError_t ec = hipStreamEndCapture(h->stream, &graph);
        if (rc) { if (graph) (void)hipGraphDestroy(graph); return rc; }
        if (ec != hipSuccess || !graph) return fail(h, RSREC_ERR_DEVICE, "hipStreamEndCapture failed: %s", hipGetErrorString(ec));
        const hipError_t ei = hipGraphInstantiate(&h->graph_exec, graph, nullptr, nullptr, 0);
        (void)hipGraphDestroy(graph);
        if (ei != hipSuccess) { h->graph_exec = nullptr; return fail(h, RSREC_ERR_DEVICE, "hipGraphInstantiate failed: %s", hipGetErrorString(ei)); }
        h->graph_key = key;
    }
    HIPCK(h, hipGraphLaunch(h->graph_exec, h->stream));
    return RSREC_OK;
}

int rotate_resident_coef(rsrec_t* h, RecursionCall& RC, double2* dA, double2* dB, int c0, int nb, int lld) {
    hipEvent_t r0 = next_event(h);
    k_rotate_coef<<<dim3(2 * (lld - 1), nb), 256, 0, h->stream>>>(dA, dB, h->d_rot.as<double2>() + (size_t)c0 * BLK, lld);
    HIPCK(h, hipGetLastError());
    RC.rot_ev.emplace_back(r0, next_event(h));
    return RSREC_OK;
}
int recursion_end(rsrec_t* h, const RecursionCall& RC, int res_kind, int lld, bool seeded) {
    hipEvent_t ev_end = next_event(h);
    const int rc = finish_status(h);
    finish_timing(h, RC.ev_begin, ev_end, RC.hop_ev);
    for (auto& pr : RC.rot_ev) h->t_rot_ms += ev_ms(pr.first, pr.second);
    if (rc) return rc;
    h->res_kind = res_kind; h->res_n = RC.nchains; h->res_lld = lld; h->res_seeded = seeded;
    return RSREC_OK;
}

template <class L, bool MFMA>
int run_block_lanczos(rsrec_t* h, int nchains, int nseed, const int32_t* seed_atoms, const double* seed_coef, int lld, double* a_b, double* b2_b,
                      const double* rot = nullptr ) {
    const int kk = h->kk;
    const bool hoh = h->hoh != 0;
    const int nsteps = lld - 1;
    if (rot && !MFMA) return fail(h, RSREC_ERR_ARG, "local-axis recursion needs the matrix-core kernel set (option kernels = 0 or 2)");
    RecursionCall RC = recursion_call(h, MFMA, nchains, nseed, nsteps, rot);
    const int ci = RC.ci, ntau = h->nmax + h->ntype;
    const size_t cstride = (size_t)lld * BLK, orth_lds = TILE_ATOMS * BLK * sizeof(double2);
    drop_resident(h);
    HIPCK(h, h->d_coefA.reserve((size_t)nchains * lld * BLK * sizeof(double2)));
    HIPCK(h, h->d_coefB.reserve((size_t)nchains * lld * BLK * sizeof(double2)));
    if (rot) {
        HIPCK(h, h->d_rot.reserve((size_t)nchains * BLK * sizeof(double2)));
        XFER(xfer_h2d(h, h->d_rot.p, rot, (size_t)nchains * BLK * sizeof(double2)));
    }
    const bool oop = MFMA && h->opt_orth_oop != 0 && h->opt_orth3 != 2;
    const int nvec = MFMA ? (oop && hoh ? 5 : 4) : (hoh ? 3 : 2);
    const bool use_v1 = !MFMA || hoh || oop;
    const size_t gram_groups = ((size_t)kk + 7 * (size_t)(h->nmax + h->ntype) + 8 + GROUP - 1) / GROUP;
    const bool gram_eligible = MFMA && ci && !hoh && !rot && h->ntype == 1 && h->nmax == 0 && h->ham_hermitian && h->opt_s5_split != 3 &&
                               RC.op->single_class(0) >= 0 && (h->opt_nblk <= 0 || 2 * h->opt_nblk >= S5_GRAM_MAXW) &&
                               s5_gram_folds((long)gram_groups, h->opt_s5_gram_min);
    const size_t gram_cstride = gram_eligible ? gram_groups * 2 * S5_GRAM_DOUBLES : 0;
    XFER(recursion_begin(h, RC, nvec, use_v1 ? -1 : 1, nseed, gram_cstride));
    const int B = RC.B, nblk = RC.nblk;
    HIPCK(h, h->d_frags.reserve((size_t)B * 3 * 27 * 64 * sizeof(double)));
    HIPCK(h, h->d_bmats.reserve((size_t)B * 2 * BLK * sizeof(double2)));
    const size_t gram_elems = (size_t)B * 256 * 1296;
    double *pmn = h->d_vec[1].as<double>(), *hpsi = h->d_vec[2].as<double>();
    double2* partial = h->d_partial.as<double2>();
    double *gpartial = h->d_partial.as<double>(), *bfrags = h->d_frags.as<double>();
    HIPCK(h, hipFuncSetAttribute(reinterpret_cast<const void*>(k_orth<L>), hipFuncAttributeMaxDynamicSharedMemorySize, TILE_ATOMS * BLK * (int)sizeof(double2)));
    h->hop_fuses_a = MFMA ? 0 : 1;

    for (int c0 = 0; c0 < nchains; c0 += B) {
        const int nb = std::min(B, nchains - c0);
        double2* dA = h->d_coefA.as<double2>() + (size_t)c0 * cstride;
        double2* dB = h->d_coefB.as<double2>() + (size_t)c0 * cstride;
        RecursionBatch bt;
        XFER(recursion_batch(h, RC, seed_atoms, seed_coef, c0, nb, bt));
        const ChainView &CV = bt.CV, &CVp = bt.CVp;
        const rsrec_handle::RegionEntry* RE = h->cur_entry;
        auto fold_at = [&](int lv) -> int {
            if (!gram_eligible || !RE || lv < 0 || lv >= (int)RE->hop_max.size()) return 0;
            if (!s5_gram_folds(RE->hop_max[lv] / GROUP, h->opt_s5_gram_min)) return 0;
            return s5_gram_folds(RE->hop_min[lv] / GROUP, h->opt_s5_gram_min) ? 2 : 1;
        };
        for (int ll = 0; ll < nsteps; ++ll) { const int f = fold_at(ll + 1); h->n_gram_folded += f > 0; h->n_gram_all += f == 2; h->n_gram_levels += 1; }
        auto enqueue_levels = [&]() -> int {
            XFER(clear_vectors(h, RC, nb, MFMA && !hoh ? 2 : -1));
            HIPCK(h, hipMemsetAsync(dA, 0, (size_t)nb * cstride * sizeof(double2), h->stream));
            HIPCK(h, hipMemsetAsync(dB, 0, (size_t)nb * cstride * sizeof(double2), h->stream));
            if (MFMA) HIPCK(h, hipMemsetAsync(bfrags, 0, (size_t)nb * 3 * 27 * 64 * sizeof(double), h->stream));
            double *psi = h->d_vec[0].as<double>(), *t2 = h->d_vec[3].as<double>();
            double* t3 = oop ? h->d_vec[hoh ? 4 : 1].as<double>() : nullptr;
            seed_chains(h, RC, nb, psi);
            k_set_identity<<<nb, 256, 0, h->stream>>>(dB, cstride);
            if (MFMA) k_uscheme_init<<<nb, 256, 0, h->stream>>>(h->d_bmats.as<double2>(), bfrags, ci);
            const dim3 grid(nblk, nb);
            SideReduce SR{RC.side};
            double* gp_b = SR.side ? gpartial + gram_elems : gpartial;
            for (int ll = 0; ll < nsteps; ++ll) {
                const int lv_final = hoh ? 2 * ll + 2 : ll + 1;
                if (MFMA) {
                    const int folds = fold_at(lv_final);
                    const GramFold GF{folds ? CV.cum : nullptr, RC.nlev, h->opt_s5_gram_min};
                    XFER(apply_h(h, RC, bt, ll + 1, psi, hpsi, pmn, bt.la_extra, ntau, S5Epilogue(),
                                 folds ? S5Gram{h->d_gram.as<double>(), gram_cstride, h->opt_s5_gram_min} : S5Gram()));
                    const dim3 gl = level_grid(h, bt.grid_mf, lv_final);
                    if (folds < 2) k_mfma_adot<<<gl, MF_WAVES * 64, 0, h->stream>>>(CVp, lv_final, kk, psi, hpsi, gpartial, GF);
                    if (folds) k_gram_groupsum<<<gl, 384, 0, h->stream>>>(GF, lv_final, h->d_gram.as<double>(), gram_cstride, gpartial);
                    int n2 = gl.x; const double* p2 = presum(h, gpartial, nb, n2, 1296);
                    XFER(side_reduce_wait(h, SR));
                    k_reduce_a_u<<<nb, 1024, 0, h->stream>>>(p2, n2, dA + (size_t)ll * BLK, cstride, h->d_bmats.as<double2>(), bfrags, ci);
                    if (h->opt_orth3 == 2) k_mfma_orth3w<<<gl, MF_WAVES * 64, 0, h->stream>>>(CVp, lv_final, kk, hpsi, psi, t2, bfrags, gp_b);
                    else k_mfma_orth3<<<gl, MF_WAVES * 64, 0, h->stream>>>(CVp, lv_final, kk, hpsi, psi, t2, bfrags, gp_b, t3);
                    hipStream_t st; XFER(side_reduce_begin(h, SR, st));
                    n2 = gl.x; p2 = presum(h, gp_b, nb, n2, 1296, st, SR.side ? 1 : 0);
                    k_reduce_b_u<<<nb, 1024, 0, st>>>(p2, n2, dB + (size_t)(ll + 1) * BLK, cstride, h->d_bmats.as<double2>(), bfrags, h->d_status.as<int>(), ci);
                    XFER(side_reduce_end(h, SR));
                    if (oop) { double* f = t2; t2 = psi; psi = t3; t3 = f; }
                    else std::swap(psi, t2);
                    continue;
                }
                XFER((valu_apply_h<AM_LANCZOS, AM_HOH_LANCZOS>(h, RC, bt, ll + 1, psi, psi, pmn, hpsi)));
                k_reduce_a<<<nb, 1024, 0, h->stream>>>(partial, nblk, dA + (size_t)ll * BLK, cstride);
                k_orth<L><<<grid, NTHREADS, orth_lds, h->stream>>>(CV, lv_final, psi, pmn, (const double*)nullptr, dA + (size_t)ll * BLK, cstride, partial);
                k_reduce_b_eig<<<nb, 1024, 0, h->stream>>>(partial, nblk, dB + (size_t)(ll + 1) * BLK, cstride, h->d_bmats.as<double2>(), h->d_status.as<int>());
                k_update<L><<<grid, NTHREADS, 0, h->stream>>>(CV, lv_final, psi, pmn, h->d_bmats.as<double2>());
            }
            HIPCK(h, hipGetLastError());
            return side_reduce_wait(h, SR);
        };
        const bool use_graph = MFMA && nchains <= B && ((h->opt_graph == 1 && nchains <= 8) || h->opt_graph >= 2) && getenv("RSREC_NO_GRAPH") == nullptr;
        if (!use_graph) XFER(enqueue_levels());
        else {
            if (ci) HIPCK(h, h->d_s5queue.reserve((size_t)nb * 16 * sizeof(int)));
            const Spmm5Operator& OP = *RC.op;
            std::vector<uintptr_t> key = {(uintptr_t)1 , (uintptr_t)nb, (uintptr_t)lld, (uintptr_t)nseed, (uintptr_t)hoh, (uintptr_t)ci, (uintptr_t)(rot != nullptr), (uintptr_t)kk,
                                          (uintptr_t)h->cur_order, (uintptr_t)h->cur_cum, (uintptr_t)bt.ostride, (uintptr_t)OP.d_frag, (uintptr_t)OP.d_meta, (uintptr_t)OP.ntr,
                                          (uintptr_t)h->s4_op.frag_set(0), (uintptr_t)h->s4_op.meta_set(0), (uintptr_t)h->d_nbr.p, (uintptr_t)h->d_nbr5.p, (uintptr_t)h->d_iz.p,
                                          (uintptr_t)h->d_partial.p, (uintptr_t)h->d_partial2.p, (uintptr_t)h->d_frags.p, (uintptr_t)dA, (uintptr_t)dB, (uintptr_t)h->d_bmats.p,
                                          (uintptr_t)h->d_status.p, (uintptr_t)h->d_seed.p, (uintptr_t)h->d_seedcoef.p, (uintptr_t)h->d_la_extra.p, (uintptr_t)h->d_s5queue.p,
                                          (uintptr_t)h->cur_entry, (uintptr_t)h->p2_slot, (uintptr_t)OP.single_class(0), (uintptr_t)OP.spin_mixing,
                                          (uintptr_t)h->lattice_epoch, (uintptr_t)OP.sched_epoch, (uintptr_t)h->nslots, (uintptr_t)h->nmax, (uintptr_t)h->ntype, (uintptr_t)h->hslots,
                                          (uintptr_t)B, (uintptr_t)h->n_cu, (uintptr_t)h->d_gram.p, (uintptr_t)gram_eligible};
            for (int v = 0; v < nvec; ++v) key.push_back((uintptr_t)h->d_vec[v].p);
            for (const OptionEntry& o : OPTIONS)
                if (o.member != &rsrec_handle::opt_graph) key.push_back((uintptr_t)(h->*o.member));
            XFER(replay_level_loop(h, key, enqueue_levels));
            h->n_hop_launch += (double)nsteps * (hoh ? 2 : 1);
        }
        if (rot && lld > 1) XFER(rotate_resident_coef(h, RC, dA, dB, c0, nb, lld));
        XFER(xfer_d2h(h, a_b + (size_t)c0 * cstride * 2, dA, (size_t)nb * cstride * sizeof(double2)));
        XFER(xfer_d2h(h, b2_b + (size_t)c0 * cstride * 2, dB, (size_t)nb * cstride * sizeof(double2)));
        HIPCK(h, hipStreamSynchronize(h->stream));
    }
    if (MFMA && h->n_gram_levels > 0 && h->n_gram_all == h->n_gram_levels) h->hop_fuses_a = 1;
    return recursion_end(h, RC, 1, lld, seed_coef != nullptr);
}

}

extern "C" int rsrec_block_lanczos_seeded(rsrec_t* h, int nchains, int nseed, const int32_t* seed_atoms, const double* seed_coef, int lld,
                                          double* a_b, double* b2_b) {
    int rc = check_ready(h, "rsrec_block_lanczos");
    if (rc) return rc;
    if (nchains < 0 || nseed < 1 || lld < 1 || !a_b || !b2_b || (nchains > 0 && !seed_atoms)) return fail(h, RSREC_ERR_ARG, "rsrec_block_lanczos: bad argument");
    XFER(check_seeds(h, "rsrec_block_lanczos", seed_atoms, (size_t)nchains * nseed, 1));
    HIPCK(h, hipSetDevice(h->device));
    reset_timing(h);
    if (nchains == 0) return RSREC_OK;
    if (matrix_core_set(h)) return run_block_lanczos<LayoutRM, true>(h, nchains, nseed, seed_atoms, seed_coef, lld, a_b, b2_b);
    return run_block_lanczos<LayoutCM, false>(h, nchains, nseed, seed_atoms, seed_coef, lld, a_b, b2_b);
}

extern "C" int rsrec_block_lanczos(rsrec_t* h, int nsites, const int32_t* seed_atoms, int lld, double* a_b, double* b2_b) {
    return rsrec_block_lanczos_seeded(h, nsites, 1, seed_atoms, nullptr, lld, a_b, b2_b);
}

namespace {

int build_local_axis_operator(rsrec_t* h) {
    if (h->s5_la_ok) return RSREC_OK;
    const int ntau = h->nmax + h->ntype, nfs = h->nslots + 1, nset = h->hoh ? 2 : 1;
    const size_t B = 2 * (size_t)BLK;
    std::vector<const double*> blk((size_t)nset * ntau * nfs, nullptr);
    std::vector<double> dense(B, 1.0), neg((size_t)ntau * h->nslots * B, 0.0);
    for (int tau = 0; tau < ntau; ++tau) {
        for (int s = 0; s < h->nslots; ++s) {
            const double* src = tau < h->nmax ? h->host_hall.data() + B * (s + (size_t)h->hslots * tau) : h->host_ee.data() + B * (s + (size_t)h->hslots * (tau - h->nmax));
            blk[((size_t)0 * ntau + tau) * nfs + s] = src;
            if (nset > 1) {
                const double* so = tau < h->nmax ? h->host_hallo.data() + B * (s + (size_t)h->hslots * tau) : h->host_eeo.data() + B * (s + (size_t)h->hslots * (tau - h->nmax));
                double* d = neg.data() + B * (s + (size_t)h->nslots * tau);
                for (size_t e = 0; e < B; ++e) d[e] = -so[e];
                if (s == 0) for (int q = 0; q < NB; ++q) d[2 * (q + NB * q)] += 1.0;
                blk[((size_t)1 * ntau + tau) * nfs + s] = d;
            }
// ... 1633 lines not shown
void whole_lattice_apply_h(WholeLatticeCall& W, const double* in, double* out, S5Epilogue epi = S5Epilogue()) {
    if (!W.h->hoh) { whole_lattice_spmm(W, W.h->s5_op, 0, in, out, nullptr, epi); return; }
    whole_lattice_spmm(W, W.h->s5_op, 0, in, W.hps, nullptr);
    whole_lattice_spmm(W, W.h->s5_op, 1, W.hps, out, in, epi);
}
void whole_lattice_apply_v_prepare(WholeLatticeCall& W, const double* in) {
    if (W.h->hoh) whole_lattice_spmm(W, W.h->nmax > 0 ? W.h->kubo_hbulk : W.h->s5_op, 0, in, W.p1, nullptr);
}
void whole_lattice_apply_v_prepared(WholeLatticeCall& W, const Spmm5Operator& vop, const double* in, double* out) {
    if (!W.h->hoh) { whole_lattice_spmm(W, vop, 0, in, out, nullptr); return; }
    whole_lattice_spmm(W, vop, 0, in, W.p2, nullptr);
    whole_lattice_spmm(W, vop, 1, W.p1, out, W.p2);
}
void whole_lattice_apply_v(WholeLatticeCall& W, const Spmm5Operator& vop, const double* in, double* out) {
    whole_lattice_apply_v_prepare(W, in);
    whole_lattice_apply_v_prepared(W, vop, in, out);
}

struct ChebyshevStepper {
    double *old, *cur, *spare;
    void rotate(int n) {
        if (n == 1) std::swap(old, cur);
        else { double* o = spare; spare = old; old = cur; cur = o; }
    }
    void step(WholeLatticeCall& W, int n, double a, double b) {
        if (n == 0) return;
        rotate(n);
        whole_lattice_apply_h(W, old, cur, cheb_epilogue(n == 1, old, spare, a, b));
    }
};

int whole_lattice_end(rsrec_t* h, WholeLatticeCall& W, bool rest_is_own_spans = false) {
    hipEvent_t ev_end = next_event(h);
    HIPCK(h, hipStreamSynchronize(h->stream));
    HIPCK(h, hipGetLastError());
    if (!W.timed) { h->t_total_ms = ev_ms(W.ev_begin, ev_end); return RSREC_OK; }
    finish_timing(h, W.ev_begin, ev_end, W.hop_ev);
    h->n_hop_launch = (double)W.hop_ev.size();
    if (!rest_is_own_spans) return RSREC_OK;
    h->t_rest_ms = 0;
    for (auto& pr : W.rest_ev) h->t_rest_ms += ev_ms(pr.first, pr.second);
    const double fan = (double)std::count_if(h->nbr.begin(), h->nbr.end(), [](int nbr) { return nbr >= 0; });
    h->n_block_mult = fan * W.chain_launches;
    h->n_atom_steps = (double)h->kk * W.chain_launches;
    return RSREC_OK;
}

struct KuboPlan {
    int cond_ll = 0, n_cu = 0, nout = 1;
    int nin = 1, setgroup = 1;
    bool diag = false, resident = false;
    int nchunk = 0, lchunk = 0, nbv = 0;
    int ksteps_total = 0, nbn_max = 0;
    size_t velems = 0, sstride = 0, lstride = 0;
    size_t part_image = 0;
    size_t bytes[5] = {0, 0, 0, 0, 0};
    int ksplit_for(int lc) const {
        const long blocks = (long)(diag ? (lc + KD_T - 1) / KD_T : (lc * NB + KG_BLK - 1) / KG_BLK) * nbn_max;
        long ksp = (12L * (diag ? 3 : 8) * n_cu + blocks - 1) / std::max(1L, blocks);
        ksp = std::min<long>({ksp, 64, std::max(1, ksteps_total / 64)});
        return (int)std::max<long>(8, (ksp + 7) / 8 * 8);
    }
    double *work = nullptr, *Lm = nullptr, *Rm = nullptr;
    double2 *part = nullptr, *mu = nullptr;
    enum { PSIREF = 0, Y = 1 , L0 = 4, HPS = 6, P1 = 7, P2 = 8, L1 = 9 };
    double* vec(int v) const { return work + (size_t)v * sstride; }
    double* Lslot(int q) const { return Lm + (size_t)q * lstride; }
    double* Rslot(int j, int q) const { return Rm + ((size_t)j * nchunk + q) * sstride; }
};

constexpr int KUBO_CHAINS_MAX = 8;
constexpr int KUBO_SETGROUP_MAX = 3;
constexpr int KUBO_SETGROUP_DEFAULT = 2;

int kubo_plan(rsrec_t* h, int nin, int nout, int setgroup, int nvec, int cond_ll, bool diag, KuboPlan& P) {
    const int kk = h->kk;
    P.diag = diag; P.nout = nout; P.nin = nin;
    const int nset = nin * nout;
    P.setgroup = std::max(1, std::min({setgroup, KUBO_SETGROUP_MAX, nset}));
    P.cond_ll = cond_ll; P.n_cu = h->n_cu; P.velems = (size_t)(kk + 1) * BLD;
    P.nchunk = std::min(cond_ll, 64);
    size_t free_b = 0, total_b = 0;
    HIPCK(h, hipMemGetInfo(&free_b, &total_b));
    size_t reusable = 0;
    for (int v = 0; v < 6; ++v) reusable += h->d_vec[v].bytes;
    for (auto& kb : h->d_kubo) reusable += kb.bytes;
    const double budget = 0.9 * (double)(free_b + reusable);
    P.ksteps_total = (int)((NB * (size_t)kk + 3) / 4);
    P.nbn_max = diag ? (P.nchunk + KD_T - 1) / KD_T : (P.nchunk * NB + KG_BLK - 1) / KG_BLK;
    const double mu_bytes = (double)cond_ll * cond_ll * (diag ? NB : BLK) * 16.0;
    auto part_bytes = [&](int lc) {
        if (diag) return (double)P.ksplit_for(lc) * ((lc + KD_T - 1) / KD_T) * KD_T * (double)P.nbn_max * KD_T * NB * 16.0;
        return (double)P.ksplit_for(lc) * ((lc * NB + KG_BLK - 1) / KG_BLK) * KG_BLK * (double)P.nbn_max * KG_BLK * 16.0; };
    auto need_for = [&](int lc, int nv) { return (11.0 * nin + lc + (double)nset * P.nchunk) * nv * P.velems * 8 + P.setgroup * part_bytes(lc) + (double)nv * nset * mu_bytes; };
    int lchunk = cond_ll;
    if (h->opt_kubo_lchunk > 0) lchunk = (int)std::min<long>(cond_ll, h->opt_kubo_lchunk);
    int nbv = (int)std::min<long>({(long)nvec, h->opt_kubo_vbatch > 0 ? h->opt_kubo_vbatch : KUBO_CHAINS_MAX, (long)(KUBO_CHAINS_MAX / nin)});
    while (nbv > 1 && need_for(lchunk, nbv) > budget) --nbv;
    while (lchunk > 1 && need_for(lchunk, nbv) > budget) lchunk = (lchunk + 1) / 2;
    if (need_for(lchunk, nbv) > budget)
        return fail(h, RSREC_ERR_DEVICE, "rsrec_kubo_moments: %.1f GB needed for one left vector at a time on %d atoms, %.1f GB free", need_for(1, 1) * 1e-9, kk, free_b * 1e-9);
    P.lchunk = lchunk; P.nbv = nbv; P.lstride = (size_t)nbv * P.velems; P.sstride = (size_t)nin * P.lstride;
    P.bytes[0] = 11 * P.sstride * 8; P.bytes[1] = (size_t)lchunk * P.lstride * 8; P.bytes[2] = (size_t)nout * P.nchunk * P.sstride * 8;
    P.resident = diag && need_for(lchunk, nbv) + (double)(nvec - nbv) * nset * mu_bytes <= budget;
    P.part_image = (size_t)part_bytes(lchunk) / 16;
    P.bytes[3] = P.setgroup * P.part_image * 16; P.bytes[4] = (size_t)(P.resident ? nvec : nbv) * nset * (size_t)mu_bytes;
    return RSREC_OK;
}

int kubo_reserve(rsrec_t* h, KuboPlan& P) {
    for (int v = 0; v < 6; ++v) h->d_vec[v].release();
    for (int q = 0; q < 5; ++q) if (h->d_kubo[q].bytes < P.bytes[q]) h->d_kubo[q].release();
    for (int q = 0; q < 5; ++q)
        if (h->d_kubo[q].reserve(P.bytes[q]) != hipSuccess) {
            for (auto& kb : h->d_kubo) kb.release();
            return fail(h, RSREC_ERR_DEVICE, "rsrec_kubo_moments: out of device memory");
        }
    P.work = h->d_kubo[0].as<double>(); P.Lm = h->d_kubo[1].as<double>(); P.Rm = h->d_kubo[2].as<double>();
    P.part = h->d_kubo[3].as<double2>(); P.mu = h->d_kubo[4].as<double2>();
    HIPCK(h, hipMemsetAsync(P.Lm, 0, P.bytes[1], h->stream));
    HIPCK(h, hipMemsetAsync(P.Rm, 0, P.bytes[2], h->stream));
    HIPCK(h, hipMemsetAsync(P.work, 0, P.bytes[0], h->stream));
    return RSREC_OK;
}

struct KuboSeeds { int nseed; const int32_t* atoms; const double* coef; };

void whole_vector_seeds(const KuboSeeds& S, int iv, std::vector<int>& s0, std::vector<double>& c0) {
    s0.clear(); c0.clear();
    for (int k = 0; k < S.nseed; ++k) {
        const size_t e = (size_t)iv * S.nseed + k;
        if (S.atoms[e] == 0) continue;
        s0.push_back(S.atoms[e] - 1); c0.push_back(S.coef[2 * e]); c0.push_back(S.coef[2 * e + 1]);
    }
}

template <class L>
int seed_whole_vectors(rsrec_t* h, const char* who, const KuboSeeds& S, int iv0, int nb, double* vec, size_t velems) {
    std::vector<int> s0; std::vector<double> c0;
    for (int c = 0; c < nb; ++c) {
        whole_vector_seeds(S, iv0 + c, s0, c0);
        if (s0.empty()) return fail(h, RSREC_ERR_ARG, "%s: vector %d has no seed", who, iv0 + c + 1);
        XFER(xfer_h2d(h, h->d_seed.p, s0.data(), s0.size() * 4));
        XFER(xfer_h2d(h, h->d_seedcoef.p, c0.data(), c0.size() * 8));
        k_seed<L><<<1, 64, 0, h->stream>>>(vec + (size_t)c * velems, velems, h->d_seed.as<int>(), h->d_seedcoef.as<double2>(), (int)s0.size());
        HIPCK(h, hipStreamSynchronize(h->stream));
    }
    return RSREC_OK;
}

int kubo_seed_batch(rsrec_t* h, const KuboPlan& P, const KuboSeeds& S, int iv0, int nb) {
    double* psiref = P.vec(KuboPlan::PSIREF);
    HIPCK(h, hipMemsetAsync(psiref, 0, P.sstride * 8, h->stream));
    return seed_whole_vectors<LayoutCI>(h, "rsrec_kubo_moments", S, iv0, nb, psiref, P.velems);
}

int kubo_left_chunk(WholeLatticeCall& W, const KuboPlan& P, int m0, double a, double b) {
    rsrec_t* h = W.h;
    const int ml = std::min(P.lchunk, P.cond_ll - m0);
    const size_t cpy = ((size_t)W.SD.nchains * P.velems - BLD) * 8;
    double *l0 = P.vec(KuboPlan::L0), *l1 = P.vec(KuboPlan::L1);
    for (int m = m0; m < m0 + ml; ++m) {
        double* out = P.Lslot(m - m0);
        const double* prev1 = m - 1 >= m0 ? P.Lslot(m - 1 - m0) : l1;
        const double* prev2 = m - 2 >= m0 ? P.Lslot(m - 2 - m0) : (m - 2 == m0 - 1 ? l1 : l0);
        if (m == 0) HIPCK(h, hipMemcpyAsync(out, P.vec(KuboPlan::PSIREF), cpy, hipMemcpyDeviceToDevice, h->stream));
        else if (m == 1) whole_lattice_apply_h(W, prev1, out, cheb_epilogue(true, prev1, nullptr, a, b));
        else whole_lattice_apply_h(W, prev1, out, cheb_epilogue(false, prev1, prev2, a, b));
    }
    if (m0 + ml < P.cond_ll) {
        if (ml >= 2) HIPCK(h, hipMemcpyAsync(l0, P.Lslot(ml - 2), cpy, hipMemcpyDeviceToDevice, h->stream));
        else HIPCK(h, hipMemcpyAsync(l0, l1, cpy, hipMemcpyDeviceToDevice, h->stream));
        HIPCK(h, hipMemcpyAsync(l1, P.Lslot(ml - 1), cpy, hipMemcpyDeviceToDevice, h->stream));
    }
    return RSREC_OK;
}

int kubo_ksplit(const rsrec_t* h, const KuboPlan& P, int per_cu, int nbm, int nbn) {
    int ksplit = 8;
    const long slots = (long)per_cu * h->n_cu, cap = std::min<long>(P.ksplit_for(P.lchunk), std::max(8, P.ksteps_total / 64 / 8 * 8));
    double best = 0.0;
    for (long c = 8; c <= cap; c += 8) {
        const long tasks = (long)nbm * nbn * c, rounds = (tasks + slots - 1) / slots;
        const double eff = (double)tasks / (double)(rounds * slots) * (rounds >= 3 ? 1.0 : 0.9);
        if (eff > best + 1e-9) { best = eff; ksplit = (int)c; }
    }
    return ksplit;
}

template <class MuOff>
int kubo_contract_diag(WholeLatticeCall& W, const KuboPlan& P, int nb, int s_lo, int ns, int m0, int n, MuOff&& mu_off) {
    rsrec_t* h = W.h;
    const int nl = n % P.nchunk, n0 = n - nl, nv = nl + 1, mv = std::min(P.lchunk, P.cond_ll - m0);
    const int nbm = (mv + KD_T - 1) / KD_T, nbn = (nv + KD_T - 1) / KD_T;
// ... 337 lines not shown
    const bool mu_dev = is_device_ptr(mu_diag), out_dev = is_device_ptr(opt);
    const size_t mu_set = (size_t)NB * L * L, out_set = (size_t)NB * nw * nf;
    const size_t pt_l = (size_t)lp * ep * sizeof(double2), part_l = (size_t)nti * ntj * nf * KO_NDIAG * sizeof(double2);
    const int nl_max = (int)std::max<size_t>(1, std::min<size_t>(NB, OPT_WORK_BYTES / (pt_l + part_l)));
    const size_t o_ft = (size_t)lp * ep, o_fr = o_ft + (size_t)nf * ep, o_w = o_fr + 2 * (size_t)nf * nb, o_ene = o_w + L, o_fermi = o_ene + nen,
                 o_live = o_fermi + nf, n0 = o_live + ((size_t)nti * ntj + 1) / 2;
    const size_t o_out = mu_dev ? 0 : 2 * mu_set, n4 = o_out + (out_dev ? 0 : 2 * out_set * nset);
    const size_t want[5] = {n0 * sizeof(double), (size_t)nl_max * lp * lp * sizeof(double2), nl_max * pt_l, nl_max * part_l, n4 * sizeof(double)};
    const bool keep_diag = h->kubo_diag_nvec != 0;
    for (int k = 0; k < 5; ++k) XFER(reserve_beside_kubo(h, h->d_opt[k], want[k], keep_diag));
    double* T = h->d_opt[0].as<double>();
    XFER(xfer_h2d(h, T + o_w, w.data(), (size_t)L * sizeof(double)));
    XFER(xfer_h2d(h, T + o_ene, ene, (size_t)nen * sizeof(double)));
    XFER(xfer_h2d(h, T + o_fermi, fermi, (size_t)nf * sizeof(double)));
    double2* d_fr = reinterpret_cast<double2*>(T + o_fr);
    int* d_live = reinterpret_cast<int*>(T + o_live);
    double* stage = h->d_opt[4].as<double>();
    double2* out = out_dev ? reinterpret_cast<double2*>(opt) : reinterpret_cast<double2*>(stage + o_out);
    std::vector<std::pair<hipEvent_t, hipEvent_t>> kev;
    hipEvent_t e_begin = next_event(h);
    k_opt_basis<<<(ep + 255) / 256, 256, 0, h->stream>>>(nen, ep, L, lp, nf, T + o_ene, T + o_w, T + o_fermi, sc.a, sc.b, temperature, T, T + o_ft);
    k_opt_fermi_range<<<(nb * nf + 255) / 256, 256, 0, h->stream>>>(nen, ep, nf, T + o_ft, d_fr);
    k_opt_tiles<<<(nti * ntj + 255) / 256, 256, 0, h->stream>>>(nen, ep, nw, nf, nti, ntj, d_fr, d_live);
    HIPCK(h, hipGetLastError());
    kev.emplace_back(e_begin, next_event(h));
    for (int s = 0; s < nset; ++s) {
        const double2* src;
        if (mu_dev) src = reinterpret_cast<const double2*>(mu_diag) + mu_set * s;
        else {
            if (s > 0) HIPCK(h, hipStreamSynchronize(h->stream));
            XFER(xfer_h2d(h, stage, mu_diag + 2 * mu_set * s, 2 * mu_set * sizeof(double)));
            src = reinterpret_cast<const double2*>(stage);
        }
        for (int l0 = 0; l0 < NB; l0 += nl_max) {
            const int nl = std::min(nl_max, NB - l0);
            const size_t gelems = (size_t)nl * lp * lp;
            hipEvent_t c0 = next_event(h);
            k_opt_gather<<<(int)std::min<size_t>(4096, (gelems + 255) / 256), 256, 0, h->stream>>>(src, l0, nl, L, lp, h->d_opt[1].as<double2>());
            k_opt_project<<<dim3((unsigned)((ep + 255) / 256), (unsigned)(lp / KO_TM), (unsigned)nl), 256, 0, h->stream>>>(
                ep, lp, lk, T, h->d_opt[1].as<double2>(), h->d_opt[2].as<double2>());
            k_opt_fused<<<dim3((unsigned)((ntj + 3) / 4), (unsigned)nti, (unsigned)nl), 256, 0, h->stream>>>(
                nen, ep, lp, lk, nw, nf, nti, ntj, T, h->d_opt[2].as<double2>(), T + o_ft, d_live, h->d_opt[3].as<double2>());
            k_opt_reduce<<<(int)(((size_t)nl * nw * nf + 255) / 256), 256, 0, h->stream>>>(nw, nf, nti, ntj, l0, nl, pref, d_live, h->d_opt[3].as<double2>(),
                                                                                            out + out_set * s);
            HIPCK(h, hipGetLastError());
            kev.emplace_back(c0, next_event(h));
        }
    }
    hipEvent_t e_end = next_event(h);
    HIPCK(h, hipStreamSynchronize(h->stream));
    if (!out_dev) XFER(xfer_d2h(h, opt, out, out_set * nset * sizeof(double2)));
    h->t_total_ms = ev_ms(e_begin, e_end);
    for (auto& pr : kev) h->t_rest_ms += ev_ms(pr.first, pr.second);
    return RSREC_OK;
}

}

extern "C" int rsrec_kubo_optical(rsrec_t* h, int nset, int cond_ll, const double* mu_diag, int nen, const double* ene, double energy_min, double energy_max,
                                  int nw, int nfermi, const double* fermi, double temperature, double* opt) {
    if (!h) return RSREC_ERR_ARG;
    return kubo_optical_run(h, nset, cond_ll, mu_diag, nen, ene, energy_min, energy_max, nw, nfermi, fermi, temperature, opt);
}

extern "C" int rsrec_orbital_moments(rsrec_t* h, int nseeds, const int32_t* seed_atoms, int lld, double a, double b, const double* cr, double alat,
                                     double* mu_orb, double* mu_seed) {
    XFER(check_ready(h, "rsrec_orbital_moments"));
    if (nseeds < 0 || lld < 1 || a == 0.0 || !cr || !mu_orb || (nseeds > 0 && !seed_atoms)) return fail(h, RSREC_ERR_ARG, "rsrec_orbital_moments: bad argument");
    XFER(check_seeds(h, "rsrec_orbital_moments", seed_atoms, (size_t)nseeds, 1));
    if (!h->s5_built) return fail(h, RSREC_ERR_ARG, "rsrec_orbital_moments: lattice has too many neighbour slots for the SpMM kernel");
    HIPCK(h, hipSetDevice(h->device));
    reset_timing(h);
    std::fill(mu_orb, mu_orb + 2 * (size_t)BLK * lld, 0.0);
    if (nseeds == 0) return RSREC_OK;
    const int kk = h->kk;
    const bool hoh = h->hoh != 0;
    if (hoh) XFER(build_plain_operator(h));
    const Spmm5Operator& plain = hoh ? h->orb_plain : h->s5_op;
    const size_t velems = (size_t)(kk + 1) * BLD;
    const int nvec = hoh ? 5 : 4;
    BatchPlan bp;
    XFER(plan_batch(h, nseeds, nvec, velems / 2, bp));
    const int B = bp.batch;
    for (int v = 0; v < nvec; ++v) HIPCK(h, h->d_vec[v].reserve((size_t)B * velems * sizeof(double)));
    XFER(reserve_partials(h, B, 2 * (size_t)B * 256 * 1296 * sizeof(double)));
    HIPCK(h, h->d_seed.reserve((size_t)B * 4));
    HIPCK(h, h->d_seedcoef.reserve((size_t)B * sizeof(double2)));
    HIPCK(h, h->d_scal.reserve((size_t)3 * kk * sizeof(double)));
    HIPCK(h, h->d_zsqr.reserve((size_t)B * lld * BLK * sizeof(double2)));
    XFER(xfer_h2d(h, h->d_scal.p, cr, (size_t)3 * kk * sizeof(double)));
    WholeLatticeCall W;
    XFER(whole_lattice_begin(h, W, B, true));
    W.hps = hoh ? h->d_vec[4].as<double>() : nullptr;
    W.ev_begin = next_event(h);
    double2* d_out = h->d_zsqr.as<double2>();
    const size_t ostr = (size_t)lld * BLK;
    std::vector<double> host_out;
    for (int c0 = 0; c0 < nseeds; c0 += B) {
        const int nb = std::min(B, nseeds - c0);
        std::vector<int> s0;
        std::vector<double> one;
        stage_seeds(seed_atoms, nullptr, c0, nb, 1, s0, one);
        XFER(xfer_h2d(h, h->d_seed.p, s0.data(), s0.size() * 4));
        XFER(xfer_h2d(h, h->d_seedcoef.p, one.data(), one.size() * 8));
        whole_lattice_batch(W, nb, true);
        double* left = h->d_vec[0].as<double>();
        ChebyshevStepper V{h->d_vec[1].as<double>(), h->d_vec[2].as<double>(), h->d_vec[3].as<double>()};
        for (int v = 0; v < nvec; ++v) HIPCK(h, hipMemsetAsync(h->d_vec[v].p, 0, (size_t)nb * velems * sizeof(double), h->stream));
        k_seed<LayoutCI><<<nb, 64, 0, h->stream>>>(V.cur, velems, h->d_seed.as<int>(), h->d_seedcoef.as<double2>(), 1);
        whole_lattice_spmm(W, plain, 0, V.cur, left, nullptr, cheb_epilogue(true, V.cur, nullptr, a, b));
        k_orb_left<<<dim3(std::min(kk, 1024), nb), 256, 0, h->stream>>>(kk, velems, h->d_seed.as<int>(), h->d_scal.as<double>(), alat, reinterpret_cast<double2*>(left));
        const dim3 grid_mf(std::max(1, std::min(mfma_workgroups_per_chain(h, nb), (W.CV.ostride / GROUP + MF_WAVES - 1) / MF_WAVES)), nb);
        const dim3 gl = level_grid(h, grid_mf, 0);
        for (int n = 0; n < lld; ++n) {
            V.step(W, n, a, b);
            k_mfma_adot<<<gl, MF_WAVES * 64, 0, h->stream>>>(W.CV, 0, kk, left, V.cur, h->d_partial.as<double>());
            int n2 = gl.x;
            const double* p2 = presum(h, h->d_partial.as<double>(), nb, n2, 1296);
            k_reduce_gram_out<<<nb, 1024, 0, h->stream>>>(p2, n2, d_out + (size_t)n * BLK, ostr, 1);
        }
        HIPCK(h, hipGetLastError());
        host_out.resize((size_t)nb * ostr * 2);
        XFER(xfer_d2h(h, host_out.data(), d_out, host_out.size() * sizeof(double)));
        for (int q = 0; q < nb; ++q) {
            const double* src = host_out.data() + (size_t)q * ostr * 2;
            for (size_t e = 0; e < ostr * 2; ++e) mu_orb[e] += src[e];
            if (mu_seed) memcpy(mu_seed + (size_t)(c0 + q) * ostr * 2, src, ostr * 2 * sizeof(double));
        }
    }
    XFER(whole_lattice_end(h, W));
    drop_resident(h);
    return RSREC_OK;
}

extern "C" int rsrec_apply_operator(rsrec_t* h, int vel, const double* v_op, const double* vo_op, const double* psi_in, double* psi_out, double a, double b) {
    XFER(check_ready(h, "rsrec_apply_operator"));
    if (!psi_in || !psi_out || (vel != 1 && a == 0.0) || (vel == 1 && (!v_op || (h->hoh && !vo_op))) || vel < 0 || vel > 2) return fail(h, RSREC_ERR_ARG, "rsrec_apply_operator: bad argument");
    if (!h->s5_built) return fail(h, RSREC_ERR_ARG, "rsrec_apply_operator: lattice has too many neighbour slots for the SpMM kernel");
    HIPCK(h, hipSetDevice(h->device));
    reset_timing(h);
    const int kk = h->kk;
    const size_t velems = (size_t)(kk + 1) * BLD, nd = (size_t)kk * BLD;
    if (vel == 1) { XFER(build_kubo_operator(h, h->kubo_op[0], v_op, vo_op)); if (h->hoh && h->nmax > 0) XFER(build_kubo_hbulk(h)); }
    if (vel == 2 && h->hoh) XFER(build_plain_operator(h));
    for (int v = 0; v < 6; ++v) HIPCK(h, h->d_vec[v].reserve(velems * 8));
    for (int v = 0; v < 6; ++v) HIPCK(h, hipMemsetAsync(h->d_vec[v].p, 0, velems * 8, h->stream));
    WholeLatticeCall W;
    XFER(whole_lattice_begin(h, W, 1, false));
    double* in = h->d_vec[0].as<double>(); double* out = h->d_vec[1].as<double>(); double* tmp = h->d_vec[2].as<double>();
    W.hps = h->d_vec[3].as<double>(); W.p1 = h->d_vec[4].as<double>(); W.p2 = h->d_vec[5].as<double>();
    XFER(xfer_h2d(h, tmp, psi_in, nd * 8));
    W.ev_begin = next_event(h);
    k_block_transpose<true><<<std::min(kk, 2048), 384, 0, h->stream>>>(kk, reinterpret_cast<const double2*>(tmp), reinterpret_cast<double2*>(in));
    if (vel == 1) whole_lattice_apply_v(W, h->kubo_op[0], in, out);
    else {
        if (vel == 2 && h->hoh) whole_lattice_spmm(W, h->orb_plain, 0, in, tmp, nullptr);
        else whole_lattice_apply_h(W, in, tmp);
        k_cheb_combine<true><<<(int)std::min<size_t>(4096, (nd + 255) / 256), 256, 0, h->stream>>>(nd, tmp, in, nullptr, out, a, b);
    }
    k_block_transpose<false><<<std::min(kk, 2048), 384, 0, h->stream>>>(kk, reinterpret_cast<const double2*>(out), reinterpret_cast<double2*>(tmp));
    XFER(whole_lattice_end(h, W));
    XFER(xfer_d2h(h, psi_out, tmp, nd * 8));
    return RSREC_OK;
}

namespace {

struct LatticeCall {
    int nchains, lld, ngroup;
    KuboSeeds S;
    const int32_t* group;
    double a, b;
    double* m_g;
};

struct LatticeBatchLists { std::vector<int> list, seg_off, split_off; std::vector<double> weight, bound; int pstride = 1; };
void lattice_lists(const rsrec_t* h, const LatticeCall& A, int c0, int nb, LatticeBatchLists& T) {
    const int kk = h->kk, ng = A.ngroup;
    T.list.assign((size_t)nb * kk, 0); T.weight.assign((size_t)2 * nb * kk, 0.0);
    T.seg_off.assign((size_t)nb * (ng + 1), 0); T.split_off.assign((size_t)nb * (ng + 1), 0); T.bound.assign(nb, 0.0);
    T.pstride = 1;
    std::vector<int> s0, placed(kk), fill(ng);
    std::vector<double> cf;
    for (int c = 0; c < nb; ++c) {
        whole_vector_seeds(A.S, c0 + c, s0, cf);
        std::fill(placed.begin(), placed.end(), -1);
        for (size_t k = 0; k < s0.size(); ++k) placed[s0[k]] = (int)k;
        int *goff = T.seg_off.data() + (size_t)c * (ng + 1), *soff = T.split_off.data() + (size_t)c * (ng + 1);
        double norm2 = 0.0;
        for (int j = 0; j < kk; ++j) {
            if (placed[j] < 0) continue;
            norm2 += cf[2 * placed[j]] * cf[2 * placed[j]] + cf[2 * placed[j] + 1] * cf[2 * placed[j] + 1];
            const int g = A.group ? A.group[j] : 1;
            if (g > 0) goff[g] += 1;
        }
        for (int g = 0; g < ng; ++g) {
            soff[g + 1] = soff[g] + lattice_splits(goff[g + 1]);
            fill[g] = goff[g];
            goff[g + 1] += goff[g];
        }
        for (int j = 0; j < kk; ++j) {
            const int g = A.group ? A.group[j] : 1;
            if (placed[j] < 0 || g <= 0) continue;
            const size_t pos = (size_t)c * kk + fill[g - 1]++;
            T.list[pos] = j; T.weight[2 * pos] = cf[2 * placed[j]]; T.weight[2 * pos + 1] = -cf[2 * placed[j] + 1];
        }
        T.pstride = std::max(T.pstride, soff[ng]);
        T.bound[c] = 1000.0 * std::max(1.0, norm2);
    }
}

void lattice_step_valu(WholeLatticeCall& W, ChebyshevStepper& Y, const DevProblem& P, int nblk, int n, double a, double b, double* tmp) {
    if (n == 0) return;
    rsrec_t* h = W.h;
    Y.rotate(n);
    const bool first = n == 1;
    const dim3 grid(nblk, W.SD.nchains);
    ApplyArgs G{};
    G.partial = h->d_partial.as<double2>(); G.a = a; G.b = b; G.in = Y.old; G.cur = Y.old; G.v0 = first ? Y.old : Y.spare; G.out = Y.cur; G.level = 0;
    auto timed = [&](auto&& launch) {
        hipEvent_t e0 = next_event(h);
        launch();
        W.hop_ev.emplace_back(e0, next_event(h));
        W.chain_launches += W.SD.nchains;
    };
    if (!h->hoh) {
        timed([&] { if (first) k_apply<AM_CHEB1, LayoutCM><<<grid, NTHREADS, 0, h->stream>>>(P, W.CV, G); else k_apply<AM_CHEBN, LayoutCM><<<grid, NTHREADS, 0, h->stream>>>(P, W.CV, G); });
        return;
    }
    G.out = tmp;
    timed([&] { k_apply<AM_STORE, LayoutCM><<<grid, NTHREADS, 0, h->stream>>>(P, W.CV, G); });
    G.in = tmp; G.v1 = tmp; G.out = Y.cur;
    timed([&] { if (first) k_apply<AM_HOH_CHEB1, LayoutCM><<<grid, NTHREADS, 0, h->stream>>>(P, W.CV, G); else k_apply<AM_HOH_CHEBN, LayoutCM><<<grid, NTHREADS, 0, h->stream>>>(P, W.CV, G); });
}

template <bool MFMA>
int run_lattice(rsrec_t* h, const char* who, const LatticeCall& A) {
    using L = typename std::conditional<MFMA, LayoutCI, LayoutCM>::type;
    const bool hoh = h->hoh != 0;
    const int kk = h->kk, ng = A.ngroup, napply = 2 * A.lld + 1, nmom = 2 * A.lld + 2, nvec = hoh ? 4 : 3;
    const size_t velems = (size_t)(kk + 1) * BLD, mstride = (size_t)nmom * BLK, nimg = (size_t)A.nchains * ng;
    const size_t pmax = (size_t)kk / LATTICE_SPLIT_ATOMS + ng + 1;
    drop_resident(h);
    release_kubo_buffers(h, true, true);
    HIPCK(h, h->d_mu.reserve(nimg * mstride * sizeof(double2)));
    size_t free_b = 0, total_b = 0, reusable = h->d_lat_tab.bytes + h->d_lat_w.bytes + h->d_lat_part.bytes + (MFMA ? 0 : h->d_partial.bytes + h->d_partial2.bytes);
    HIPCK(h, hipMemGetInfo(&free_b, &total_b));
    for (int v = 0; v < nvec; ++v) reusable += h->d_vec[v].bytes;
    const double per_chain = (double)nvec * velems * 8 + (double)kk * 20 + (double)pmax * BLK * 16 + (MFMA ? 0.0 : 3.0 * 256 * 2 * 1296 * 8) + 4096;
    const double budget = 0.85 * (double)(free_b + reusable);
    int nbv = (int)std::min<long>(A.nchains, h->opt_lattice_vbatch > 0 ? std::min<long>(h->opt_lattice_vbatch, 64) : KUBO_CHAINS_MAX);
    while (nbv > 1 && per_chain * nbv > budget) --nbv;
    if (per_chain * nbv > budget) return fail(h, RSREC_ERR_DEVICE, "%s: %.1f GB needed for one chain on %d atoms, %.1f GB free", who, per_chain * 1e-9, kk, free_b * 1e-9);
    for (int v = 0; v < nvec; ++v) HIPCK(h, h->d_vec[v].reserve((size_t)nbv * velems * sizeof(double)));
    if (!MFMA) XFER(reserve_partials(h, nbv, (size_t)nbv * 256 * 2 * 1296 * sizeof(double)));
    const int nblk = (int)std::max<long>(1, std::min<long>({h->opt_nblk > 0 ? h->opt_nblk : std::max<long>(2048 / nbv, 16), 256, (kk + TILE_ATOMS - 1) / TILE_ATOMS}));
    HIPCK(h, h->d_status.reserve(64));
    HIPCK(h, hipMemsetAsync(h->d_status.p, 0, 64, h->stream));
    HIPCK(h, h->d_seed.reserve((size_t)A.S.nseed * 4));
    HIPCK(h, h->d_seedcoef.reserve((size_t)A.S.nseed * sizeof(double2)));
    const size_t n_list = (size_t)nbv * kk, n_off = (size_t)nbv * (ng + 1);
    HIPCK(h, h->d_lat_tab.reserve((n_list + 2 * n_off) * sizeof(int)));
    HIPCK(h, h->d_lat_w.reserve(n_list * sizeof(double2) + (size_t)nbv * sizeof(double)));
    HIPCK(h, h->d_lat_part.reserve((size_t)nbv * pmax * BLK * sizeof(double2)));
    int *d_list = h->d_lat_tab.as<int>(), *d_seg = d_list + n_list, *d_split = d_seg + n_off;
    double2* d_w = h->d_lat_w.as<double2>();
    double* d_bound = reinterpret_cast<double*>(d_w + n_list);
    double2* partial = h->d_lat_part.as<double2>();
    double2* mu = h->d_mu.as<double2>();
    WholeLatticeCall W;
    XFER(whole_lattice_begin(h, W, nbv, true, MFMA));
    W.hps = hoh ? h->d_vec[3].as<double>() : nullptr;
    const DevProblem P = make_problem(h);
    W.ev_begin = next_event(h);
    LatticeBatchLists T;
    for (int c0 = 0; c0 < A.nchains; c0 += nbv) {
        const int nb = std::min(nbv, A.nchains - c0);
        whole_lattice_batch(W, nb, false);
        lattice_lists(h, A, c0, nb, T);
        if ((size_t)T.pstride > pmax) return fail(h, RSREC_ERR_DEVICE, "%s: split partials outside the planned buffer", who);
        XFER(xfer_h2d(h, d_list, T.list.data(), (size_t)nb * kk * sizeof(int)));
        XFER(xfer_h2d(h, d_seg, T.seg_off.data(), (size_t)nb * (ng + 1) * sizeof(int)));
        XFER(xfer_h2d(h, d_split, T.split_off.data(), (size_t)nb * (ng + 1) * sizeof(int)));
        XFER(xfer_h2d(h, d_w, T.weight.data(), (size_t)nb * kk * sizeof(double2)));
        XFER(xfer_h2d(h, d_bound, T.bound.data(), (size_t)nb * sizeof(double)));
        const LatticeLists LL{d_list, d_w, d_seg, d_split, kk, ng, T.pstride};
        for (int v = 0; v < nvec; ++v) HIPCK(h, hipMemsetAsync(h->d_vec[v].p, 0, (size_t)nb * velems * sizeof(double), h->stream));
        ChebyshevStepper Y{h->d_vec[0].as<double>(), h->d_vec[1].as<double>(), h->d_vec[2].as<double>()};
        XFER(seed_whole_vectors<L>(h, who, A.S, c0, nb, Y.cur, velems));
        for (int n = 0; n <= napply; ++n) {
            if (MFMA) Y.step(W, n, A.a, A.b);
            else lattice_step_valu(W, Y, P, nblk, n, A.a, A.b, h->d_vec[3].as<double>());
            hipEvent_t e0 = next_event(h);
            k_lattice_project<<<dim3(T.pstride, nb), LATTICE_THREADS, 0, h->stream>>>(LL, Y.cur, velems, partial);
            k_lattice_reduce<L><<<dim3(ng, nb, LATTICE_RWG), 64, 0, h->stream>>>(LL, partial, c0, n, nmom, mu);
            k_lattice_diverge<<<nb, LATTICE_THREADS, 0, h->stream>>>(mu, c0, n, nmom, ng, d_bound, h->d_status.as<int>());
            W.rest_ev.emplace_back(e0, next_event(h));
        }
        HIPCK(h, hipGetLastError());
    }
    if (A.m_g) {
        if (is_device_ptr(A.m_g)) HIPCK(h, hipMemcpyAsync(A.m_g, mu, nimg * mstride * sizeof(double2), hipMemcpyDeviceToDevice, h->stream));
        else XFER(xfer_d2h(h, A.m_g, mu, nimg * mstride * sizeof(double2)));
    }
    XFER(whole_lattice_end(h, W, true));
    XFER(finish_status(h));
    h->res_kind = 2; h->res_n = (int)nimg; h->res_lld = A.lld; h->res_seeded = false;
    return RSREC_OK;
}

}

extern "C" int rsrec_chebyshev_lattice(rsrec_t* h, int nchains, int nseed, const int32_t* seed_atoms, const double* seed_coef, int lld, double a, double b,
                                       int ngroup, const int32_t* group, double* m_g) {
    const char* who = "rsrec_chebyshev_lattice";
    int rc = check_ready(h, who);
    if (rc) return rc;
    if (nchains < 0 || lld < 1 || a == 0.0) return fail(h, RSREC_ERR_ARG, "%s: nchains < 0, lld < 1 or a == 0", who);
    if (nseed < 1 || nseed > h->kk) return fail(h, RSREC_ERR_ARG, "%s: nseed = %d outside 1..%d", who, nseed, h->kk);
    if (ngroup < 1 || ngroup > RSREC_LATTICE_NGROUP_MAX) return fail(h, RSREC_ERR_ARG, "%s: ngroup = %d outside 1..%d", who, ngroup, RSREC_LATTICE_NGROUP_MAX);
    if (nchains > 0 && (!seed_atoms || !seed_coef)) return fail(h, RSREC_ERR_ARG, "%s: NULL seed_atoms or seed_coef", who);
    if (!group && ngroup != 1) return fail(h, RSREC_ERR_ARG, "%s: ngroup = %d needs a group array", who, ngroup);
    if (group)
        for (int j = 0; j < h->kk; ++j)
            if (group[j] < 0 || group[j] > ngroup) return fail(h, RSREC_ERR_ARG, "%s: group(%d) = %d outside 0..%d", who, j + 1, group[j], ngroup);
    XFER(check_seeds(h, who, seed_atoms, (size_t)nchains * nseed, 0));
    for (int c = 0; c < nchains; ++c)
        if (std::all_of(seed_atoms + (size_t)c * nseed, seed_atoms + (size_t)(c + 1) * nseed, [](int32_t s) { return s == 0; }))
            return fail(h, RSREC_ERR_ARG, "%s: vector %d has no seed", who, c + 1);
    if ((size_t)nchains * ngroup > (size_t)INT32_MAX) return fail(h, RSREC_ERR_ARG, "%s: nchains * ngroup exceeds the index range", who);
    HIPCK(h, hipSetDevice(h->device));
    reset_timing(h);
    if (nchains == 0) return RSREC_OK;
    const LatticeCall A{nchains, lld, ngroup, KuboSeeds{nseed, seed_atoms, seed_coef}, group, a, b, m_g};
    return matrix_core_set(h) ? run_lattice<true>(h, who, A) : run_lattice<false>(h, who, A);
}

extern "C" int rsrec_scalar_lanczos(rsrec_t* h, int nsites, const int32_t* seed_atoms, int lld, int llmax, double* a, double* b2) {
    int rc = check_ready(h, "rsrec_scalar_lanczos");
    if (rc) return rc;
    if (nsites < 0 || lld < 1 || llmax < lld || !a || !b2 || (nsites > 0 && !seed_atoms)) return fail(h, RSREC_ERR_ARG, "rsrec_scalar_lanczos: bad argument");
    XFER(check_seeds(h, "rsrec_scalar_lanczos", seed_atoms, (size_t)nsites, 1));
    HIPCK(h, hipSetDevice(h->device));
    reset_timing(h);
    std::fill(a, a + (size_t)llmax * NB * nsites, 0.0);
    std::fill(b2, b2 + (size_t)llmax * NB * nsites, 0.0);
    if (nsites == 0) return RSREC_OK;
    if (h->nsp != 1) {
        for (size_t q = 0; q < (size_t)NB * nsites; ++q) {
            b2[q * llmax] = 1.0;
            for (int ll = 3; ll < lld; ++ll) b2[q * llmax + ll] = std::nan("");
        }
        return RSREC_OK;
    }
    const int kk = h->kk;
    const int nsteps = lld - 1;
    const int nlev = nsteps + 1;
    const size_t velems = (size_t)kk * NB;
    const int B = (int)std::min<long>(nsites, h->opt_batch > 0 ? h->opt_batch : 16);
    const int nblk = (int)std::min<long>(std::max<long>(1, (kk + TILE_ATOMS - 1) / TILE_ATOMS), 64);
    const int nch = B * NB;
    release_kubo_buffers(h, true, true);
    for (int v = 0; v < 2; ++v) HIPCK(h, h->d_vec[v].reserve((size_t)nch * velems * sizeof(double2)));
    HIPCK(h, h->d_scal.reserve((size_t)nch * (nblk + 2 * (size_t)lld) * sizeof(double) + 64));
    HIPCK(h, h->d_seed.reserve((size_t)nch * 2 * 4));
    double2* psi = h->d_vec[0].as<double2>();
    double2* pmn = h->d_vec[1].as<double2>();
    double* part = h->d_scal.as<double>();
    double* ca = part + (size_t)nch * nblk;
    double* cb = ca + (size_t)nch * lld;
    const DevProblem P = make_problem(h);
    hipEvent_t ev_begin = next_event(h);
    std::vector<double> ha((size_t)nch * lld), hb((size_t)nch * lld);
    for (int c0 = 0; c0 < nsites; c0 += B) {
        const int nb = std::min(B, nsites - c0);
        const int nc = nb * NB;
        std::vector<int> seeds0(nb), so((size_t)nc * 2);
        for (int q = 0; q < nb; ++q) {
            seeds0[q] = seed_atoms[c0 + q] - 1;
            for (int l = 0; l < NB; ++l) { so[2 * (q * NB + l)] = seeds0[q]; so[2 * (q * NB + l) + 1] = l; }
        }
        double dummy1 = 0, dummy2 = 0;
        int ostride = kk;
        rc = upload_regions(h, seeds0.data(), nb, 1, nlev, nsteps, false, false, ostride, dummy1, dummy2);
        if (rc) return rc;
        h->n_atom_steps += dummy1 * NB;
        XFER(xfer_h2d(h, h->d_seed.p, so.data(), so.size() * 4));
        HIPCK(h, hipStreamSynchronize(h->stream));
        ChainView CV;
        chain_views(h, nlev, velems, NB, ostride, CV);
        for (int v = 0; v < 2; ++v) HIPCK(h, hipMemsetAsync(h->d_vec[v].p, 0, (size_t)nc * velems * sizeof(double2), h->stream));
        HIPCK(h, hipMemsetAsync(ca, 0, (size_t)nch * 2 * lld * sizeof(double), h->stream));
        k_scalar_seed<<<nc, 64, 0, h->stream>>>(psi, velems, h->d_seed.as<int>(), cb, lld);
        const dim3 grid(nblk, nc);
        for (int ll = 0; ll < nsteps; ++ll) {
            k_scalar_hop<<<grid, NTHREADS, 0, h->stream>>>(P, CV, ll + 1, psi, pmn, part);
            k_scalar_reduce<<<nc, 64, 0, h->stream>>>(part, nblk, ca, lld, ll);
            k_scalar_orth<<<grid, NTHREADS, 0, h->stream>>>(kk, CV, ll + 1, psi, pmn, ca, lld, ll, part);
            k_scalar_reduce<<<nc, 64, 0, h->stream>>>(part, nblk, cb, lld, ll + 1);
            k_scalar_update<<<grid, NTHREADS, 0, h->stream>>>(kk, CV, ll + 1, psi, pmn, cb, lld, ll);
            h->n_hop_launch += 1;
        }
        HIPCK(h, hipGetLastError());
        XFER(xfer_d2h(h, ha.data(), ca, (size_t)nc * lld * sizeof(double)));
        XFER(xfer_d2h(h, hb.data(), cb, (size_t)nc * lld * sizeof(double)));
        HIPCK(h, hipStreamSynchronize(h->stream));
        for (int q = 0; q < nc; ++q)
            for (int ll = 0; ll < lld; ++ll) {
                a[(size_t)llmax * ((size_t)c0 * NB + q) + ll] = ha[(size_t)q * lld + ll];
                b2[(size_t)llmax * ((size_t)c0 * NB + q) + ll] = hb[(size_t)q * lld + ll];
            }
    }
    hipEvent_t ev_end = next_event(h);
    HIPCK(h, hipStreamSynchronize(h->stream));
    h->t_total_ms = ev_ms(ev_begin, ev_end);
    return RSREC_OK;
}
```

rslmtoasa_amd/recursion.py:

```python
import ctypes as C
import os
from dataclasses import dataclass, field

import numpy as np

from . import _lib


@dataclass
class Control:
    lld: int = 21
    llsp: int = 0
    nsp: int = 2
    recur: str = "block"


@dataclass
class Energy:
    energy_min: float = -1.0
    energy_max: float = 1.0


@dataclass
class Lattice:
    nn: np.ndarray
    iz: np.ndarray
    irec: np.ndarray
    nmax: int = 0
    ntype: int = 1
    ijpair: np.ndarray = None
    cr: np.ndarray = None

    @property
    def kk(self):
        return self.nn.shape[0]

    @property
    def nrec(self):
        return len(self.irec)


@dataclass
class Hamiltonian:
    ee: np.ndarray
    lsham: np.ndarray
    eeo: np.ndarray = None
    enim: np.ndarray = None
    hall: np.ndarray = None
    hallo: np.ndarray = None
    hoh: bool = False
    local_axis: bool = False


def site_partition(rank, nprocs, nsites):
    s, e = C.c_int(), C.c_int()
    _lib.lib().rsrec_site_partition(rank, nprocs, nsites, C.byref(s), C.byref(e))
    return s.value, e.value


def chebyshev_scaling(energy_min, energy_max):
    a = (energy_max - energy_min) / float(np.float32(2) - np.float32(0.3))
    b = (energy_max + energy_min) / 2
    return a, b


def _fc(a, dtype):
    return np.asfortranarray(np.asarray(a, dtype=dtype))


def _ptr(a):
    return None if a is None else a.ctypes.data_as(C.c_void_p)


class Recursion:

    def __init__(self, hamiltonian, lattice, control, energy=None, device=0, rank=0, nprocs=1):
        self.hamiltonian, self.lattice, self.control, self.en = hamiltonian, lattice, control, energy or Energy()
        self.rank, self.nprocs = rank, nprocs
        self._L = _lib.lib()
        self._h = C.c_void_p()
        rc = self._L.rsrec_create(C.byref(self._h), device)
        if rc != 0:
            raise _lib.RsrecError(rc, "rsrec_create failed (no usable gfx950 device? there is no CPU fallback)")
        self.restore_to_default()
        self.update_lattice()
        self.update_hamiltonian()

    def close(self):
        if getattr(self, "_h", None) is not None and self._h.value:
            self._L.rsrec_destroy(self._h)
            self._h = C.c_void_p()

    def __del__(self):
        try:
            self.close()
        except Exception:
            pass

    def _check(self, rc):
        if rc != 0:
            buf = C.create_string_buffer(512)
            self._L.rsrec_last_error(self._h, buf, 512)
            raise _lib.RsrecError(rc, buf.value.decode(errors="replace"))

    def set_option(self, key, value):
        self._check(self._L.rsrec_set_option(self._h, key.encode(), int(value)))


    def timing(self):
        out = (C.c_double * 14)()
        self._L.rsrec_get_timing(self._h, out, 14)
        keys = ("total_ms", "hop_ms", "hop_launches", "atom_steps", "block_multiplies", "rest_ms", "host_ms", "hop_fuses_a", "hop_mfma_flop", "hop_required_flop",
                "operator_arrays_from_device", "octet_launches", "rotate_ms", "gram_folded_launches")
        return dict(zip(keys, list(out)))

    def restore_to_default(self):
        lat, ctl = self.lattice, self.control
        llmax = max(ctl.llsp, ctl.lld)
        nrec = lat.nrec
        njij = 0 if lat.ijpair is None else len(lat.ijpair)
        nsites = nrec if njij == 0 else 4 * njij
        self.a = np.zeros((llmax, 18, nrec, 3), np.float64, order="F")
        self.b2 = np.zeros((llmax, 18, nrec, 3), np.float64, order="F")
        self.a_b = np.zeros((18, 18, ctl.lld, nsites), np.complex128, order="F")
        self.b2_b = np.zeros((18, 18, ctl.lld, nsites), np.complex128, order="F")
        self.mu_n = np.zeros((18, 18, 2 * ctl.lld + 2, nsites), np.complex128, order="F")
        self.mu_ng = np.zeros_like(self.mu_n)

    def update_lattice(self):
        lat = self.lattice
        self._nn = _fc(lat.nn, np.int32)
        self._iz = _fc(lat.iz, np.int32)
        self._check(self._L.rsrec_set_lattice(self._h, lat.kk, self._nn.shape[1], _ptr(self._nn), _ptr(self._iz), int(lat.nmax), int(lat.ntype)))
        if lat.cr is not None:
            cr = _fc(lat.cr, np.float64)
            assert cr.shape == (3, lat.kk)
            self._check(self._L.rsrec_set_positions(self._h, _ptr(cr)))

    def update_hamiltonian(self):
        ham = self.hamiltonian
        keep = {}
        for k in ("ee", "lsham", "eeo", "enim", "hall", "hallo"):
            v = getattr(ham, k)
            keep[k] = None if v is None else _fc(v, np.complex128)
        self._ham_keep = keep
        self._check(self._L.rsrec_set_hamiltonian(self._h, keep["ee"].shape[2], int(bool(ham.hoh)), int(self.control.nsp),
                                                  _ptr(keep["ee"]), _ptr(keep["lsham"]), _ptr(keep["eeo"]), _ptr(keep["enim"]),
                                                  _ptr(keep["hall"]), _ptr(keep["hallo"])))

    def _assemble(self, part, hmag, nbr_type, obarm):
        hoh = bool(self.hamiltonian.hoh)
        hm = _fc(hmag, np.complex128)
        assert hm.ndim == 5 and hm.shape[:2] == (9, 9) and hm.shape[3] == 4, "hmag is (9,9,nslots,4,ncls)"
        nslots, ncls = hm.shape[2], hm.shape[4]
        ty = ob = None
        ntype = 0
        if hoh:
            ty, ob = _fc(nbr_type, np.int32), _fc(obarm, np.complex128)
            assert ty.shape == (nslots, ncls) and ob.shape[:2] == (18, 18)
            ntype = ob.shape[2]
        blocks = np.zeros((18, 18, nslots, ncls), np.complex128, order="F")
        blocks_o = np.zeros_like(blocks) if hoh else None
        self._check(self._L.rsrec_assemble_blocks(self._h, part, ncls, nslots, int(hoh), _ptr(hm), _ptr(ty), _ptr(ob), ntype, _ptr(blocks), _ptr(blocks_o)))
        return blocks, blocks_o

    def build_bulkham(self, hmag, nbr_type=None, obarm=None):
        self.hamiltonian.ee, eeo = self._assemble(0, hmag, nbr_type, obarm)
        if eeo is not None:
            self.hamiltonian.eeo = eeo

    def build_locham(self, hmag, nbr_type=None, obarm=None):
        self.hamiltonian.hall, hallo = self._assemble(1, hmag, nbr_type, obarm)
        if hallo is not None:
            self.hamiltonian.hallo = hallo

    def _my_sites(self):
        start, end = site_partition(self.rank, self.nprocs, self.lattice.nrec)
        return start, end, np.ascontiguousarray(self.lattice.irec[start - 1:end], dtype=np.int32)

    def recur_b(self):
        lld = self.control.lld
        start, end, seeds = self._my_sites()
        n = len(seeds)
        a_b = np.zeros((18, 18, lld, n), np.complex128, order="F")
        b2_b = np.zeros_like(a_b)
        self._check(self._L.rsrec_block_lanczos(self._h, n, _ptr(seeds), lld, _ptr(a_b), _ptr(b2_b)))
        self.a_b[:, :, :, :n] = a_b
        self.b2_b[:, :, :, :n] = b2_b
        d = np.arange(18)
        self.a[:lld, :, :n, 0] = a_b[d, d].real.transpose(1, 0, 2)
# ... 286 lines not shown
```

Before: 70790.

## Skip loads of unwritten shells in orth3 and add skewed vector arena

```diff
diff --git a/include/rsrec.h b/include/rsrec.h
--- a/include/rsrec.h
+++ b/include/rsrec.h
@@ -167,6 +167,7 @@
 int rsrec_comm_destroy(rsrec_t *h);
 
 int rsrec_set_option(rsrec_t *h, const char *key, long value);
+long rsrec_get_vec_skew(const rsrec_t *h);
 int rsrec_get_timing(rsrec_t *h, double *out, int n);
 
 #ifdef __cplusplus
diff --git a/rslmtoasa_amd/_lib.py b/rslmtoasa_amd/_lib.py
--- a/rslmtoasa_amd/_lib.py
+++ b/rslmtoasa_amd/_lib.py
@@ -72,6 +72,7 @@
     "rsrec_last_error": (C.c_int, [C.c_void_p, C.c_char_p, C.c_size_t]),
     "rsrec_set_option": (C.c_int, [C.c_void_p, C.c_char_p, C.c_long]),
     "rsrec_get_timing": (C.c_int, [C.c_void_p, C.POINTER(C.c_double), C.c_int]),
+    "rsrec_get_vec_skew": (C.c_long, [C.c_void_p]),
 }
 
 
diff --git a/rslmtoasa_amd/csrc/kernels_uscheme.hpp b/rslmtoasa_amd/csrc/kernels_uscheme.hpp
--- a/rslmtoasa_amd/csrc/kernels_uscheme.hpp
+++ b/rslmtoasa_amd/csrc/kernels_uscheme.hpp
@@ -59,12 +59,17 @@
 __global__ __launch_bounds__(MF_WAVES * 64, 1) void k_mfma_orth3(ChainView CV, int level, int zero_block, const double* __restrict__ tvec,
                                                                 const double* __restrict__ ucur, double* uprev,
                                                                 const double* __restrict__ tabs, double* partial ,
-                                                                double* unext = nullptr ) {
+                                                                double* unext = nullptr ,
+                                                                int level_cur = INT32_MAX ,
+                                                                int level_prev = INT32_MAX , int store = 1 ) {
     __shared__ double lds[MF_WAVES * 1296];
     const int chain = blockIdx.y;
     const int lane = threadIdx.x & 63;
     const int wave = __builtin_amdgcn_readfirstlane(threadIdx.x >> 6);
     const int ngroups = CV.count_of(chain, level) / GROUP;
+    const bool prefixes = CV.obase[(chain / CV.cpo) * CV.nlev + level] == 0;
+    auto written_end = [&](int lv) { return (!prefixes || lv >= CV.nlev) ? INT32_MAX : (lv < 0 ? 0 : CV.count_of(chain, lv)); };
+    const int end_cur = written_end(level_cur), end_prev = written_end(level_prev);
     const int* order = CV.order_of(chain, level);
     const size_t vo = (size_t)chain * CV.vstride;
     const double* tv = tvec + vo;
@@ -83,30 +88,35 @@
     const int nbx = active_workgroups(ngroups);
     GroupWalk w((int)blockIdx.x < nbx ? ngroups : 0, wave, nbx);
     const int ntile = (w.g < w.end) ? ((w.end - w.g + w.step - 1) / w.step) * 9 : 0;
-    struct TileAtoms { int s0, a_lo, a_hi; };
+    struct TileAtoms { int s0, a_lo, a_hi, pos ; };
     auto tile_atoms = [&](int it) {
         it = min(it, ntile - 1);
-        const int* __restrict__ grp = order + (size_t)(w.g + (it / 9) * w.step) * GROUP;
         TileAtoms t;
+        t.pos = (w.g + (it / 9) * w.step) * GROUP;
+        const int* __restrict__ grp = order + (size_t)t.pos;
         t.s0 = (16 * (it % 9)) / 18;
         t.a_lo = grp[t.s0];
         t.a_hi = grp[min(t.s0 + 1, GROUP - 1)];
         return t;
     };
-    auto tile_row = [&](const TileAtoms& t, int rho) {
-        const bool hi = rho >= 18 * (t.s0 + 1);
-        const int a = hi ? t.a_hi : t.a_lo;
+    auto atoms_row = [&](int s0, int a_lo, int a_hi, int rho) {
+        const bool hi = rho >= 18 * (s0 + 1);
+        const int a = hi ? a_hi : a_lo;
         RowRef R;
         R.valid = a >= 0;
-        R.off = (unsigned)BLD * (unsigned)(R.valid ? a : zero_block) + 36u * (unsigned)(rho - 18 * (t.s0 + (hi ? 1 : 0)));
+        R.off = (unsigned)BLD * (unsigned)(R.valid ? a : zero_block) + 36u * (unsigned)(rho - 18 * (s0 + (hi ? 1 : 0)));
         return R;
+    };
+    auto tile_row = [&](const TileAtoms& t, int rho) {
+        return atoms_row(t.s0, t.a_lo, t.a_hi, rho);
     };
     auto load_tile = [&](int it, U3Operands& a, U3Operands& c, U3Operands& p) {
         const TileAtoms t = tile_atoms(it);
-        const RowRef ra = tile_row(t, 16 * (min(it, ntile - 1) % 9) + l15);
-        u3_load(a, tv, ra.off, l4);
-        u3_load(c, uc, ra.off, l4);
-        u3_load(p, up, ra.off, l4);
+        const int rho = 16 * (min(it, ntile - 1) % 9) + l15;
+        const bool zc = t.pos >= end_cur, zp = t.pos >= end_prev;
+        u3_load(a, tv, tile_row(t, rho).off, l4);
+        u3_load(c, uc, atoms_row(t.s0, zc ? -1 : t.a_lo, zc ? -1 : t.a_hi, rho).off, l4);
+        u3_load(p, up, atoms_row(t.s0, zp ? -1 : t.a_lo, zp ? -1 : t.a_hi, rho).off, l4);
     };
     struct Pending { double4_t ca, cb; double cr; TileAtoms ta; int mt; };
     Pending P;
@@ -115,10 +125,10 @@
 #pragma unroll
         for (int j = 0; j < 4; ++j) {
             const RowRef rs = tile_row(P.ta, 16 * P.mt + l4 + 4 * j);
-            if (rs.valid) { st_stream(uo + rs.off + l15, (double)P.ca[j]); st_stream(uo + rs.off + 16 + l15, (double)P.cb[j]); }
+            if (rs.valid && store) { st_stream(uo + rs.off + l15, (double)P.ca[j]); st_stream(uo + rs.off + 16 + l15, (double)P.cb[j]); }
         }
         const RowRef rr = tile_row(P.ta, 16 * P.mt + 4 * lg + l4);
-        if (rr.valid) st_stream(uo + rr.off + 32 + l3, P.cr);
+        if (rr.valid && store) st_stream(uo + rr.off + 32 + l3, P.cr);
 #pragma unroll
         for (int j = 0; j < 4; ++j) {
             const double f0 = P.ca[j], f1 = P.cb[j];
diff --git a/rslmtoasa_amd/csrc/rsrec.hip b/rslmtoasa_amd/csrc/rsrec.hip
--- a/rslmtoasa_amd/csrc/rsrec.hip
+++ b/rslmtoasa_amd/csrc/rsrec.hip
@@ -45,18 +45,20 @@
 struct DevBuf {
     void* p = nullptr;
     size_t bytes = 0;
+    bool view = false;
     DevBuf() = default;
-    DevBuf(DevBuf&& o) noexcept : p(o.p), bytes(o.bytes) { o.p = nullptr; o.bytes = 0; }
-    DevBuf& operator=(DevBuf&& o) noexcept { std::swap(p, o.p); std::swap(bytes, o.bytes); return *this; }
+    DevBuf(DevBuf&& o) noexcept : p(o.p), bytes(o.bytes), view(o.view) { o.p = nullptr; o.bytes = 0; o.view = false; }
+    DevBuf& operator=(DevBuf&& o) noexcept { std::swap(p, o.p); std::swap(bytes, o.bytes); std::swap(view, o.view); return *this; }
     ~DevBuf() { release(); }
     hipError_t reserve(size_t n) {
-        if (n <= bytes) return hipSuccess;
+        if (n <= bytes && !view) return hipSuccess;
         release();
         hipError_t e = hipMalloc(&p, n);
-        if (e == hipSuccess) bytes = n;
+        if (e == hipSuccess) bytes = n; else p = nullptr;
         return e;
     }
-    void release() { if (p) (void)hipFree(p); p = nullptr; bytes = 0; }
+    void release() { if (p && !view) (void)hipFree(p); p = nullptr; bytes = 0; view = false; }
+    void point_at(void* q, size_t n) { release(); p = q; bytes = n; view = true; }
     template <class T> T* as() const { return reinterpret_cast<T*>(p); }
 };
 
@@ -124,6 +126,16 @@
     long opt_s5_waves = 8;
     long opt_sat_pct = 100;
     long opt_orth_oop = 1;
+    long opt_orth_shells = 1;
+    long opt_vec_arena = 0;
+    long opt_vec_skew = -1;
+    DevBuf d_arena;
+    struct VecArena {
+        int nvec = 0, skip = -1, slots = 0;
+        size_t vbytes = 0;
+        long kmax = 0, k = 0;
+        bool calibrate = false;
+    } arena;
     long opt_s5_split = 0;
     long opt_s5_run_min = 0;
     long opt_s5_spin_xcd = 0;
@@ -204,6 +216,9 @@
     {"s5_waves", &rsrec_handle::opt_s5_waves},
     {"s5_split", &rsrec_handle::opt_s5_split},
     {"orth_oop", &rsrec_handle::opt_orth_oop},
+    {"orth_shells", &rsrec_handle::opt_orth_shells},
+    {"vec_arena", &rsrec_handle::opt_vec_arena},
+    {"vec_skew", &rsrec_handle::opt_vec_skew},
     {"sat_pct", &rsrec_handle::opt_sat_pct},
     {"kubo_lchunk", &rsrec_handle::opt_kubo_lchunk},
     {"kubo_vbatch", &rsrec_handle::opt_kubo_vbatch},
@@ -430,6 +445,8 @@
         if (!strcmp(key, o.name)) { h->*o.member = value; return RSREC_OK; }
     return fail(h, RSREC_ERR_ARG, "unknown option '%s'", key);
 }
+
+extern "C" long rsrec_get_vec_skew(const rsrec_t* h) { return h && h->d_arena.p ? h->arena.k : -1; }
 
 extern "C" int rsrec_get_timing(rsrec_t* h, double* out, int n) {
     if (!h || !out) return RSREC_ERR_ARG;
@@ -717,19 +734,72 @@
     if (integrand) { for (auto& cb : h->d_cond) cb.release(); for (auto& cb : h->d_ctens) cb.release(); for (auto& cb : h->d_opt) cb.release(); }
 }
 
+constexpr size_t VEC_GRAIN = (size_t)64 << 10;
+constexpr long VEC_SKEW_CANDIDATES[] = {0, 1, 17, 257, 4099};
+constexpr long VEC_SKEW_MAX = 4099;
+
+size_t vec_calibrate_min_bytes() {
+    const char* e = getenv("RSREC_VEC_CALIBRATE_MIN_BYTES");
+    return e ? (size_t)strtoull(e, nullptr, 10) : (size_t)1 << 30;
+}
+long vec_arena_kmax(const rsrec_t* h, size_t vbytes) {
+    if (!h->opt_vec_arena) return -1;
+    if (h->opt_vec_skew >= 0) return h->opt_vec_skew;
+    return vbytes >= vec_calibrate_min_bytes() ? VEC_SKEW_MAX : 0;
+}
+size_t vectors_held(const rsrec_t* h, int nvec = 6) {
+    size_t n = h->d_arena.bytes;
+    for (int v = 0; v < nvec; ++v) if (!h->d_vec[v].view) n += h->d_vec[v].bytes;
+    return n;
+}
+void release_vectors(rsrec_t* h) {
+    for (int v = 0; v < 6; ++v) h->d_vec[v].release();
+    h->d_arena.release();
+    h->arena = rsrec_handle::VecArena();
+}
+void place_vectors(rsrec_t* h) {
+    const rsrec_handle::VecArena& A = h->arena;
+    const size_t stride = (A.vbytes + VEC_GRAIN - 1) / VEC_GRAIN * VEC_GRAIN + (size_t)A.k * VEC_GRAIN;
+    int slot = 0;
+    for (int v = 0; v < A.nvec; ++v)
+        if (v != A.skip) h->d_vec[v].point_at(h->d_arena.as<char>() + (size_t)slot++ * stride, A.vbytes);
+}
+int reserve_vectors(rsrec_t* h, int nvec, int skip_vec, size_t bytes, bool chain_driver = false) {
+    const long kmax = chain_driver ? vec_arena_kmax(h, bytes) : -1;
+    if (kmax >= 0) {
+        rsrec_handle::VecArena& A = h->arena;
+        const int slots = nvec - (skip_vec >= 0 && skip_vec < nvec ? 1 : 0);
+        if (h->d_arena.p && A.nvec == nvec && A.skip == skip_vec && A.vbytes >= bytes && A.kmax == kmax) return RSREC_OK;
+        release_vectors(h);
+        const size_t total = (size_t)slots * ((bytes + VEC_GRAIN - 1) / VEC_GRAIN * VEC_GRAIN + (size_t)kmax * VEC_GRAIN);
+        if (h->d_arena.reserve(total) == hipSuccess) {
+            A.nvec = nvec; A.skip = skip_vec; A.slots = slots; A.vbytes = bytes; A.kmax = kmax;
+            A.calibrate = h->opt_vec_skew < 0 && kmax > 0;
+            A.k = A.calibrate ? 0 : kmax;
+            place_vectors(h);
+            return RSREC_OK;
+        }
+        (void)hipGetLastError();
+    }
+    if (h->d_arena.p) release_vectors(h);
+    for (int v = 0; v < nvec; ++v) if (v != skip_vec) HIPCK(h, h->d_vec[v].reserve(bytes));
+    return RSREC_OK;
+}
+
 struct BatchPlan {
     int batch = 1, nblk = 1;
 };
 
-int plan_batch(rsrec_t* h, int nchains, int nvec, size_t vec_elems_per_chain, BatchPlan& bp, size_t extra_bytes_per_chain = 0) {
+int plan_batch(rsrec_t* h, int nchains, int nvec, size_t vec_elems_per_chain, BatchPlan& bp, size_t extra_bytes_per_chain = 0, bool chain_driver = false) {
     release_kubo_buffers(h, true, true);
     size_t free_b = 0, total_b = 0;
     HIPCK(h, hipMemGetInfo(&free_b, &total_b));
-    size_t reusable = 0;
-    for (int v = 0; v < 5; ++v) reusable += h->d_vec[v].bytes;
+    size_t reusable = vectors_held(h, 5);
     if (extra_bytes_per_chain) reusable += h->d_gram.bytes;
     const double per_chain = (double)nvec * vec_elems_per_chain * sizeof(double2) + (double)h->kk * 4 + 4096 + (double)extra_bytes_per_chain;
-    long cap = (long)((0.85 * (double)(free_b + reusable)) / per_chain);
+    const size_t spacers = chain_driver && h->opt_vec_arena ? (size_t)nvec * (size_t)((h->opt_vec_skew >= 0 ? h->opt_vec_skew : VEC_SKEW_MAX) + 1) * VEC_GRAIN : 0;
+    if (0.85 * (double)(free_b + reusable) <= (double)spacers) return fail(h, RSREC_ERR_DEVICE, "not enough device memory for the work vectors' arena (%.1f MB of spacers, %.1f MB free)", spacers / 1e6, free_b / 1e6);
+    long cap = (long)((0.85 * (double)(free_b + reusable) - (double)spacers) / per_chain);
     if (cap < 1) return fail(h, RSREC_ERR_DEVICE, "not enough device memory for one chain (%.1f MB needed, %.1f MB free)", per_chain / 1e6, free_b / 1e6);
     long b = h->opt_batch > 0 ? h->opt_batch : 64;
     b = std::min<long>(b, cap);
@@ -881,6 +951,9 @@
         as[c] = a_s; bm[c] = b_m;
     };
     run_threads(build_chain);
+    if (grouped)
+        for (size_t q = (size_t)2 * nb * nlev; q < (size_t)3 * nb * nlev; ++q)
+            if (cum[q] % GROUP) return fail(h, RSREC_ERR_ARG, "region lists: a level of the level-major list ends inside a group (%d entries)", cum[q]);
     double as_sum = 0.0, bm_sum = 0.0;
     for (int c = 0; c < nb; ++c) { as_sum += as[c]; bm_sum += bm[c]; }
     atom_steps += as_sum; block_mults += bm_sum;
@@ -1286,9 +1359,9 @@
     if (RC.mfma && !RC.ci) XFER(ensure_s4(h));
     RC.nvec = nvec; RC.skip_vec = skip_vec;
     BatchPlan bp;
-    XFER(plan_batch(h, RC.nchains, nvec - (skip_vec >= 0 ? 1 : 0), RC.velems / 2, bp, gram_doubles_per_chain * sizeof(double)));
+    XFER(plan_batch(h, RC.nchains, nvec - (skip_vec >= 0 ? 1 : 0), RC.velems / 2, bp, gram_doubles_per_chain * sizeof(double), true));
     const int B = RC.B = bp.batch; RC.nblk = bp.nblk;
-    for (int v = 0; v < nvec; ++v) if (v != skip_vec) HIPCK(h, h->d_vec[v].reserve((size_t)B * RC.velems * sizeof(double)));
+    XFER(reserve_vectors(h, nvec, skip_vec, (size_t)B * RC.velems * sizeof(double), true));
     if (gram_doubles_per_chain) HIPCK(h, h->d_gram.reserve((size_t)B * gram_doubles_per_chain * sizeof(double)));
     XFER(reserve_partials(h, B, (size_t)B * 256 * 2 * 1296 * sizeof(double)));
     XFER(ensure_side_stream(h));
@@ -1547,6 +1620,42 @@
         RecursionBatch bt;
         XFER(recursion_batch(h, RC, seed_atoms, seed_coef, c0, nb, bt));
         const ChainView &CV = bt.CV, &CVp = bt.CVp;
+        if (h->arena.calibrate && h->d_arena.p && MFMA && ci && h->opt_orth3 != 2 && nsteps > 0) {
+            const int lv_deep = hoh ? 2 * nsteps : nsteps;
+            const dim3 gl = level_grid(h, bt.grid_mf, lv_deep);
+            const int u_vec[3] = {0, 3, hoh ? 4 : 1}, nrot = oop ? 3 : 2;
+            hipEvent_t e0 = nullptr, e1 = nullptr;
+            HIPCK(h, hipEventCreate(&e0)); HIPCK(h, hipEventCreate(&e1));
+            HIPCK(h, hipMemsetAsync(bfrags, 0, (size_t)nb * 3 * 27 * 64 * sizeof(double), h->stream));
+            double best = 0.0; long best_k = 0;
+            for (long k : VEC_SKEW_CANDIDATES) {
+                h->arena.k = k;
+                place_vectors(h);
+                double sum = 0.0;
+                for (int r = 0; r < nrot; ++r) {
+                    double* u[3];
+                    for (int q = 0; q < 3; ++q) u[q] = h->d_vec[u_vec[(q + r) % nrot]].as<double>();
+                    float fastest = 0.f;
+                    for (int rep = 0; rep < 2; ++rep) {
+                        HIPCK(h, hipEventRecord(e0, h->stream));
+                        k_mfma_orth3<<<gl, MF_WAVES * 64, 0, h->stream>>>(CVp, lv_deep, kk, h->d_vec[2].as<double>(), u[0], u[1], bfrags, h->d_partial.as<double>(), oop ? u[2] : nullptr);
+                        HIPCK(h, hipEventRecord(e1, h->stream));
+                        HIPCK(h, hipEventSynchronize(e1));
+                        float ms = 0.f;
+                        HIPCK(h, hipEventElapsedTime(&ms, e0, e1));
+                        if (rep == 0 || ms < fastest) fastest = ms;
+                    }
+                    sum += fastest;
+                    if (getenv("RSREC_VEC_SKEW_REPORT")) fprintf(stderr, "rsrec: vec_skew k = %ld, rotation %d: %.3f ms\n", k, r, fastest);
+                }
+                if (k == VEC_SKEW_CANDIDATES[0] || sum < best) { best = sum; best_k = k; }
+            }
+            (void)hipEventDestroy(e0); (void)hipEventDestroy(e1);
+            HIPCK(h, hipGetLastError());
+            h->arena.k = best_k; h->arena.calibrate = false;
+            place_vectors(h);
+            pmn = h->d_vec[1].as<double>(); hpsi = h->d_vec[2].as<double>();
+        }
         const rsrec_handle::RegionEntry* RE = h->cur_entry;
         auto fold_at = [&](int lv) -> int {
             if (!gram_eligible || !RE || lv < 0 || lv >= (int)RE->hop_max.size()) return 0;
@@ -1581,7 +1690,13 @@
                     XFER(side_reduce_wait(h, SR));
                     k_reduce_a_u<<<nb, 1024, 0, h->stream>>>(p2, n2, dA + (size_t)ll * BLK, cstride, h->d_bmats.as<double2>(), bfrags, ci);
                     if (h->opt_orth3 == 2) k_mfma_orth3w<<<gl, MF_WAVES * 64, 0, h->stream>>>(CVp, lv_final, kk, hpsi, psi, t2, bfrags, gp_b);
-                    else k_mfma_orth3<<<gl, MF_WAVES * 64, 0, h->stream>>>(CVp, lv_final, kk, hpsi, psi, t2, bfrags, gp_b, t3);
+                    else if (h->opt_orth_shells == 0) k_mfma_orth3<<<gl, MF_WAVES * 64, 0, h->stream>>>(CVp, lv_final, kk, hpsi, psi, t2, bfrags, gp_b, t3);
+                    else {
+                        const int lv_step = hoh ? 2 : 1;
+                        const bool shells = h->opt_orth_shells != 3, last_store = h->opt_orth_shells == 2;
+                        k_mfma_orth3<<<gl, MF_WAVES * 64, 0, h->stream>>>(CVp, lv_final, kk, hpsi, psi, t2, bfrags, gp_b, t3, shells ? lv_final - lv_step : INT32_MAX,
+                                                                           shells ? lv_final - 2 * lv_step : INT32_MAX, ll == nsteps - 1 && !last_store ? 0 : 1);
+                    }
                     hipStream_t st; XFER(side_reduce_begin(h, SR, st));
                     n2 = gl.x; p2 = presum(h, gp_b, nb, n2, 1296, st, SR.side ? 1 : 0);
                     k_reduce_b_u<<<nb, 1024, 0, st>>>(p2, n2, dB + (size_t)(ll + 1) * BLK, cstride, h->d_bmats.as<double2>(), bfrags, h->d_status.as<int>(), ci);
@@ -3381,8 +3496,7 @@
     P.nchunk = std::min(cond_ll, 64);
     size_t free_b = 0, total_b = 0;
     HIPCK(h, hipMemGetInfo(&free_b, &total_b));
-    size_t reusable = 0;
-    for (int v = 0; v < 6; ++v) reusable += h->d_vec[v].bytes;
+    size_t reusable = vectors_held(h);
     for (auto& kb : h->d_kubo) reusable += kb.bytes;
     const double budget = 0.9 * (double)(free_b + reusable);
     P.ksteps_total = (int)((NB * (size_t)kk + 3) / 4);
@@ -3408,7 +3522,7 @@
 }
 
 int kubo_reserve(rsrec_t* h, KuboPlan& P) {
-    for (int v = 0; v < 6; ++v) h->d_vec[v].release();
+    release_vectors(h);
     for (int q = 0; q < 5; ++q) if (h->d_kubo[q].bytes < P.bytes[q]) h->d_kubo[q].release();
     for (int q = 0; q < 5; ++q)
         if (h->d_kubo[q].reserve(P.bytes[q]) != hipSuccess) {
@@ -3912,7 +4026,7 @@
     BatchPlan bp;
     XFER(plan_batch(h, nseeds, nvec, velems / 2, bp));
     const int B = bp.batch;
-    for (int v = 0; v < nvec; ++v) HIPCK(h, h->d_vec[v].reserve((size_t)B * velems * sizeof(double)));
+    XFER(reserve_vectors(h, nvec, -1, (size_t)B * velems * sizeof(double)));
     XFER(reserve_partials(h, B, 2 * (size_t)B * 256 * 1296 * sizeof(double)));
     HIPCK(h, h->d_seed.reserve((size_t)B * 4));
     HIPCK(h, h->d_seedcoef.reserve((size_t)B * sizeof(double2)));
@@ -3973,7 +4087,7 @@
     const size_t velems = (size_t)(kk + 1) * BLD, nd = (size_t)kk * BLD;
     if (vel == 1) { XFER(build_kubo_operator(h, h->kubo_op[0], v_op, vo_op)); if (h->hoh && h->nmax > 0) XFER(build_kubo_hbulk(h)); }
     if (vel == 2 && h->hoh) XFER(build_plain_operator(h));
-    for (int v = 0; v < 6; ++v) HIPCK(h, h->d_vec[v].reserve(velems * 8));
+    XFER(reserve_vectors(h, 6, -1, velems * 8));
     for (int v = 0; v < 6; ++v) HIPCK(h, hipMemsetAsync(h->d_vec[v].p, 0, velems * 8, h->stream));
     WholeLatticeCall W;
     XFER(whole_lattice_begin(h, W, 1, false));
@@ -4076,13 +4190,13 @@
     HIPCK(h, h->d_mu.reserve(nimg * mstride * sizeof(double2)));
     size_t free_b = 0, total_b = 0, reusable = h->d_lat_tab.bytes + h->d_lat_w.bytes + h->d_lat_part.bytes + (MFMA ? 0 : h->d_partial.bytes + h->d_partial2.bytes);
     HIPCK(h, hipMemGetInfo(&free_b, &total_b));
-    for (int v = 0; v < nvec; ++v) reusable += h->d_vec[v].bytes;
+    reusable += vectors_held(h, nvec);
     const double per_chain = (double)nvec * velems * 8 + (double)kk * 20 + (double)pmax * BLK * 16 + (MFMA ? 0.0 : 3.0 * 256 * 2 * 1296 * 8) + 4096;
     const double budget = 0.85 * (double)(free_b + reusable);
     int nbv = (int)std::min<long>(A.nchains, h->opt_lattice_vbatch > 0 ? std::min<long>(h->opt_lattice_vbatch, 64) : KUBO_CHAINS_MAX);
     while (nbv > 1 && per_chain * nbv > budget) --nbv;
     if (per_chain * nbv > budget) return fail(h, RSREC_ERR_DEVICE, "%s: %.1f GB needed for one chain on %d atoms, %.1f GB free", who, per_chain * 1e-9, kk, free_b * 1e-9);
-    for (int v = 0; v < nvec; ++v) HIPCK(h, h->d_vec[v].reserve((size_t)nbv * velems * sizeof(double)));
+    XFER(reserve_vectors(h, nvec, -1, (size_t)nbv * velems * sizeof(double)));
     if (!MFMA) XFER(reserve_partials(h, nbv, (size_t)nbv * 256 * 2 * 1296 * sizeof(double)));
     const int nblk = (int)std::max<long>(1, std::min<long>({h->opt_nblk > 0 ? h->opt_nblk : std::max<long>(2048 / nbv, 16), 256, (kk + TILE_ATOMS - 1) / TILE_ATOMS}));
     HIPCK(h, h->d_status.reserve(64));
@@ -4191,7 +4305,7 @@
     const int nblk = (int)std::min<long>(std::max<long>(1, (kk + TILE_ATOMS - 1) / TILE_ATOMS), 64);
     const int nch = B * NB;
     release_kubo_buffers(h, true, true);
-    for (int v = 0; v < 2; ++v) HIPCK(h, h->d_vec[v].reserve((size_t)nch * velems * sizeof(double2)));
+    XFER(reserve_vectors(h, 2, -1, (size_t)nch * velems * sizeof(double2)));
     HIPCK(h, h->d_scal.reserve((size_t)nch * (nblk + 2 * (size_t)lld) * sizeof(double) + 64));
     HIPCK(h, h->d_seed.reserve((size_t)nch * 2 * 4));
     double2* psi = h->d_vec[0].as<double2>();
diff --git a/rslmtoasa_amd/recursion.py b/rslmtoasa_amd/recursion.py
--- a/rslmtoasa_amd/recursion.py
+++ b/rslmtoasa_amd/recursion.py
@@ -106,6 +106,8 @@
     def set_option(self, key, value):
         self._check(self._L.rsrec_set_option(self._h, key.encode(), int(value)))
 
+    def vec_skew(self):
+        return int(self._L.rsrec_get_vec_skew(self._h))
 
     def timing(self):
         out = (C.c_double * 14)()
```

New measurement: 71010 (median of 3 runs). About the same (+0.3%).
